# Z2PackDev/TBmodels

Hardware: AMD Instinct MI355X
Metric: k-points/sec (H(k)+eig) at N_orb=64, N_R=4096 (higher is better)
Workload: dtype f64; 1 GPU; cfg2: dense N_orb=64 N_R=4096, 100000 random k-points per GPU, eigenval (H(k)+eig); kpoints_per_gpu=100000, collective=none, rccl_ranks=0, eigensolver=auto

## Files before the change

include/tbk.h:

```cpp
#ifndef TBK_H
#define TBK_H

#include <stdint.h>

#ifdef __cplusplus
extern "C" {
#endif

typedef struct tbk_model tbk_model;
typedef struct tbk_kdotp tbk_kdotp;
typedef struct tbk_comm tbk_comm;

typedef enum tbk_status {
    TBK_OK = 0,
    TBK_ERR_ARGUMENT = 1,
    TBK_ERR_DEVICE = 2,
    TBK_ERR_MEMORY = 3,
    TBK_ERR_NOT_FINITE = 4,
    TBK_ERR_NO_CONVERGENCE = 5
} tbk_status;

enum { TBK_EIG_AUTO = 0, TBK_EIG_WAVE = 1, TBK_EIG_ROCSOLVER = 2 };
enum {
    TBK_OPT_EIGENSOLVER = 1,
    TBK_OPT_K_CHUNK = 2,
    TBK_OPT_TIMING = 3,
    TBK_OPT_FOLD = 4,
    TBK_OPT_STRASSEN = 5,
    TBK_OPT_STRASSEN_LEVELS = 6
};

const char* tbk_version(void);
const char* tbk_last_error(void);
int tbk_device_count(int* count);


int tbk_model_create_dense(int device, int dim, int n_orb, int64_t n_r, const int32_t* R,
                           const double* hop, tbk_model** out);

int tbk_model_create_csr(int device, int dim, int n_orb, int64_t n_r, const int32_t* R,
                         const int64_t* r_ptr, const int32_t* row, const int32_t* col,
                         const double* val, tbk_model** out);

void tbk_model_destroy(tbk_model* m);
int tbk_model_set_option(tbk_model* m, int option, int64_t value);
int tbk_model_info(const tbk_model* m, int* device, int* dim, int* n_orb, int64_t* n_r,
                   int* is_sparse, int64_t* staged_bytes);
enum { TBK_CNT_EIGENVAL_CALLS = 0, TBK_CNT_FOLDED_CALLS = 1, TBK_CNT_FOLDED_KPOINTS = 2,
       TBK_CNT_LIBRARY_CALLS = 3,
       TBK_CNT_STRASSEN_LAUNCHES = 4,
       TBK_CNT_STRASSEN2_LAUNCHES = 5,
       TBK_CNT_COUNT = 6 };
int tbk_model_counter(tbk_model* m, int counter, int64_t* value);


int tbk_hamilton(tbk_model* m, const double* k, int64_t nk, int convention, const double* pos,
                 double* H_out);

int tbk_eigenval(tbk_model* m, const double* k, int64_t nk, double* E_out);

int tbk_eigh(tbk_model* m, const double* k, int64_t nk, int convention, const double* pos, double* E_out, double* U_out);

int tbk_eigenval_multi(tbk_model* const* handles, int n_handles, const double* k, int64_t nk, double* E_out);
int tbk_hamilton_multi(tbk_model* const* handles, int n_handles, const double* k, int64_t nk, int convention,
                       const double* pos, double* H_out);
int tbk_eigh_multi(tbk_model* const* handles, int n_handles, const double* k, int64_t nk, int convention,
                   const double* pos, double* E_out, double* U_out);

int tbk_hamilton_device(tbk_model* m, const double* d_k, int64_t nk, int convention,
                        const double* d_pos, double* d_H);
int tbk_eigenval_device(tbk_model* m, const double* d_k, int64_t nk, double* d_E);
int tbk_eigh_device(tbk_model* m, const double* d_k, int64_t nk, int convention, const double* d_pos, double* d_E,
                    double* d_U);
int tbk_eigenval_device_hint(tbk_model* m, const double* d_k, const double* h_k, int64_t nk, double* d_E);
int tbk_eigenval_check(tbk_model* m);
int tbk_synchronize(tbk_model* m);

enum { TBK_REDUCE_AUTO = 0, TBK_REDUCE_ONE_STAGE = 1, TBK_REDUCE_TWO_STAGE = 2 };
int tbk_tridiagonal_reduce(int device, int n_orb, int64_t nk, const double* H, int method, double* d, double* e,
                           double* H_reduced);

int tbk_reduce_standalone(int device, int n_orb, int64_t nk, int reps, double* us_per_matrix);

int tbk_kdotp_create(int device, int dim, int n_orb, int64_t n_p, const int32_t* powers,
                     const double* coeffs, tbk_kdotp** out);
void tbk_kdotp_destroy(tbk_kdotp* m);
int tbk_kdotp_hamilton(tbk_kdotp* m, const double* k, int64_t nk, double* H_out);
int tbk_kdotp_eigenval(tbk_kdotp* m, const double* k, int64_t nk, double* E_out);
int tbk_kdotp_eigh(tbk_kdotp* m, const double* k, int64_t nk, double* E_out, double* U_out);
int tbk_kdotp_eigenval_multi(tbk_kdotp* const* handles, int n_handles, const double* k, int64_t nk, double* E_out);
int tbk_kdotp_hamilton_multi(tbk_kdotp* const* handles, int n_handles, const double* k, int64_t nk, double* H_out);
int tbk_kdotp_eigh_multi(tbk_kdotp* const* handles, int n_handles, const double* k, int64_t nk, double* E_out, double* U_out);

int tbk_kdotp_coefficients(tbk_model* m, const double* k0, int64_t n_p, const int32_t* powers,
                           const double* prefactor, double* coeffs_out);

int tbk_device_malloc(int device, int64_t bytes, void** d_ptr);
int tbk_device_free(int device, void* d_ptr);
int tbk_memcpy_h2d(int device, void* d_dst, const void* h_src, int64_t bytes);
int tbk_memcpy_d2h(int device, void* h_dst, const void* d_src, int64_t bytes);
int tbk_device_mem_info(int device, int64_t* free_bytes, int64_t* total_bytes);

enum { TBK_T_PHASE = 0, TBK_T_HK = 1, TBK_T_EIG = 2, TBK_T_QL = 3, TBK_T_COUNT = 4 };
int tbk_get_timing(tbk_model* m, double* ms, int64_t* launches, int reset);

int tbk_comm_unique_id(void* id128);
int tbk_comm_create(int device, int world_size, int rank, const void* id128, tbk_comm** out);
void tbk_comm_destroy(tbk_comm* c);
int tbk_comm_ranks(tbk_comm* c, int* count, int* rank);
int tbk_comm_allgather_f64(tbk_comm* c, tbk_model* m, const double* d_send, double* d_recv,
                           int64_t count);
int tbk_comm_allgather_f64_overlapped(tbk_comm* c, tbk_model* m, const double* d_send, double* d_recv,
                                      int64_t count, int slot);
int tbk_comm_wait_slot(tbk_comm* c, tbk_model* m, int slot);
int tbk_comm_synchronize(tbk_comm* c);
int tbk_comm_agree(tbk_comm* c, int status, double* verdict);
int tbk_comm_prepare_gather(tbk_comm* c, int n_orb, int64_t per);

int tbk_eigenval_device_gather(tbk_comm* c, tbk_model* m, const double* d_k, const double* h_k, int64_t nk, int64_t per,
                               int host_status, double* d_all, double* d_status_all);

int tbk_mfma_f64_peak(int device, double* tflops);

#ifdef __cplusplus
}
#endif
#endif
```

tbmodels_amd/_lib.py:

```python

import ctypes
import os

import numpy as np

_HERE = os.path.dirname(os.path.abspath(__file__))
LIB_PATH = os.environ.get("TBK_LIBTBK") or os.path.join(_HERE, "libtbk.so")

TBK_OK = 0
TBK_ERR_ARGUMENT = 1
TBK_ERR_DEVICE = 2
TBK_ERR_MEMORY = 3
TBK_ERR_NOT_FINITE = 4
TBK_ERR_NO_CONVERGENCE = 5

TBK_EIG_AUTO, TBK_EIG_WAVE, TBK_EIG_ROCSOLVER = 0, 1, 2
TBK_OPT_EIGENSOLVER, TBK_OPT_K_CHUNK, TBK_OPT_TIMING, TBK_OPT_FOLD, TBK_OPT_STRASSEN, TBK_OPT_STRASSEN_LEVELS = 1, 2, 3, 4, 5, 6
TBK_REDUCE_AUTO, TBK_REDUCE_ONE_STAGE, TBK_REDUCE_TWO_STAGE = 0, 1, 2
TBK_CNT_EIGENVAL_CALLS, TBK_CNT_FOLDED_CALLS, TBK_CNT_FOLDED_KPOINTS, TBK_CNT_LIBRARY_CALLS, TBK_CNT_STRASSEN_LAUNCHES = 0, 1, 2, 3, 4
TBK_CNT_STRASSEN2_LAUNCHES = 5
TBK_T_PHASE, TBK_T_HK, TBK_T_EIG, TBK_T_QL, TBK_T_COUNT = 0, 1, 2, 3, 4
STAGE_NAMES = ("phase", "hk", "eig", "ql")

_c_int = ctypes.c_int
_c_i64 = ctypes.c_int64
_vp = ctypes.c_void_p
_pp = ctypes.POINTER(ctypes.c_void_p)

SIGNATURES = {
    "tbk_version": (ctypes.c_char_p, []),
    "tbk_last_error": (ctypes.c_char_p, []),
    "tbk_device_count": (_c_int, [ctypes.POINTER(_c_int)]),
    "tbk_model_create_dense": (_c_int, [_c_int, _c_int, _c_int, _c_i64, _vp, _vp, _pp]),
    "tbk_model_create_csr": (_c_int, [_c_int, _c_int, _c_int, _c_i64, _vp, _vp, _vp, _vp, _vp, _pp]),
    "tbk_model_destroy": (None, [_vp]),
    "tbk_model_set_option": (_c_int, [_vp, _c_int, _c_i64]),
    "tbk_model_info": (
        _c_int,
        [_vp, ctypes.POINTER(_c_int), ctypes.POINTER(_c_int), ctypes.POINTER(_c_int), ctypes.POINTER(_c_i64),
         ctypes.POINTER(_c_int), ctypes.POINTER(_c_i64)],
    ),
    "tbk_hamilton": (_c_int, [_vp, _vp, _c_i64, _c_int, _vp, _vp]),
    "tbk_eigenval": (_c_int, [_vp, _vp, _c_i64, _vp]),
    "tbk_eigenval_multi": (_c_int, [_vp, _c_int, _vp, _c_i64, _vp]),
    "tbk_hamilton_multi": (_c_int, [_vp, _c_int, _vp, _c_i64, _c_int, _vp, _vp]),
    "tbk_eigh": (_c_int, [_vp, _vp, _c_i64, _c_int, _vp, _vp, _vp]),
    "tbk_eigh_multi": (_c_int, [_vp, _c_int, _vp, _c_i64, _c_int, _vp, _vp, _vp]),
    "tbk_eigh_device": (_c_int, [_vp, _vp, _c_i64, _c_int, _vp, _vp, _vp]),
    "tbk_hamilton_device": (_c_int, [_vp, _vp, _c_i64, _c_int, _vp, _vp]),
    "tbk_eigenval_device": (_c_int, [_vp, _vp, _c_i64, _vp]),
    "tbk_eigenval_device_hint": (_c_int, [_vp, _vp, _vp, _c_i64, _vp]),
    "tbk_model_counter": (_c_int, [_vp, _c_int, ctypes.POINTER(_c_i64)]),
    "tbk_eigenval_check": (_c_int, [_vp]),
    "tbk_synchronize": (_c_int, [_vp]),
    "tbk_tridiagonal_reduce": (_c_int, [_c_int, _c_int, _c_i64, _vp, _c_int, _vp, _vp, _vp]),
    "tbk_reduce_standalone": (_c_int, [_c_int, _c_int, _c_i64, _c_int, ctypes.POINTER(ctypes.c_double)]),
    "tbk_kdotp_create": (_c_int, [_c_int, _c_int, _c_int, _c_i64, _vp, _vp, _pp]),
    "tbk_kdotp_destroy": (None, [_vp]),
    "tbk_kdotp_hamilton": (_c_int, [_vp, _vp, _c_i64, _vp]),
    "tbk_kdotp_eigenval": (_c_int, [_vp, _vp, _c_i64, _vp]),
    "tbk_kdotp_eigenval_multi": (_c_int, [_vp, _c_int, _vp, _c_i64, _vp]),
    "tbk_kdotp_hamilton_multi": (_c_int, [_vp, _c_int, _vp, _c_i64, _vp]),
    "tbk_kdotp_eigh": (_c_int, [_vp, _vp, _c_i64, _vp, _vp]),
    "tbk_kdotp_eigh_multi": (_c_int, [_vp, _c_int, _vp, _c_i64, _vp, _vp]),
    "tbk_kdotp_coefficients": (_c_int, [_vp, _vp, _c_i64, _vp, _vp, _vp]),
    "tbk_device_malloc": (_c_int, [_c_int, _c_i64, _pp]),
    "tbk_device_free": (_c_int, [_c_int, _vp]),
    "tbk_memcpy_h2d": (_c_int, [_c_int, _vp, _vp, _c_i64]),
    "tbk_memcpy_d2h": (_c_int, [_c_int, _vp, _vp, _c_i64]),
    "tbk_device_mem_info": (_c_int, [_c_int, ctypes.POINTER(_c_i64), ctypes.POINTER(_c_i64)]),
    "tbk_get_timing": (_c_int, [_vp, ctypes.POINTER(ctypes.c_double), ctypes.POINTER(_c_i64), _c_int]),
    "tbk_comm_unique_id": (_c_int, [_vp]),
    "tbk_comm_create": (_c_int, [_c_int, _c_int, _c_int, _vp, _pp]),
    "tbk_comm_destroy": (None, [_vp]),
    "tbk_comm_ranks": (_c_int, [_vp, ctypes.POINTER(_c_int), ctypes.POINTER(_c_int)]),
    "tbk_comm_allgather_f64": (_c_int, [_vp, _vp, _vp, _vp, _c_i64]),
    "tbk_comm_allgather_f64_overlapped": (_c_int, [_vp, _vp, _vp, _vp, _c_i64, _c_int]),
    "tbk_comm_wait_slot": (_c_int, [_vp, _vp, _c_int]),
    "tbk_comm_synchronize": (_c_int, [_vp]),
    "tbk_comm_agree": (_c_int, [_vp, _c_int, _vp]),
    "tbk_comm_prepare_gather": (_c_int, [_vp, _c_int, _c_i64]),
    "tbk_eigenval_device_gather": (_c_int, [_vp, _vp, _vp, _vp, _c_i64, _c_i64, _c_int, _vp, _vp]),
    "tbk_mfma_f64_peak": (_c_int, [_c_int, ctypes.POINTER(ctypes.c_double)]),
}

_LIB = None


class TbkLibraryError(RuntimeError):
    """``libtbk.so`` is missing or cannot be loaded: the product path has no CPU fallback."""


def lib():
    global _LIB
    if _LIB is None:
        if not os.path.exists(LIB_PATH):
            raise TbkLibraryError(
                "{} not found: build it with `python -c 'import __graft_entry__ as g; g.build()'` "
                "(or `make -C tbmodels_amd/csrc`). There is no CPU fallback.".format(LIB_PATH)
            )
        try:
            handle = ctypes.CDLL(LIB_PATH, mode=ctypes.RTLD_GLOBAL)
        except OSError as exc:
            raise TbkLibraryError("cannot load {}: {}".format(LIB_PATH, exc)) from exc
        for name, (restype, argtypes) in SIGNATURES.items():
            func = getattr(handle, name)
            func.restype = restype
            func.argtypes = argtypes
        _LIB = handle
    return _LIB


def last_error():
    msg = lib().tbk_last_error()
    return msg.decode("utf-8", "replace") if msg else ""


def check(status):
    if status == TBK_OK:
        return
    msg = last_error()
    if status in (TBK_ERR_ARGUMENT, TBK_ERR_NOT_FINITE):
        raise ValueError(msg)
    if status == TBK_ERR_MEMORY:
        raise MemoryError(msg)
    if status == TBK_ERR_NO_CONVERGENCE:
        raise np.linalg.LinAlgError(msg)
    raise RuntimeError(msg)


def ptr(array):
    if array is None:
        return None
    assert array.flags.c_contiguous
    return array.__array_interface__["data"][0]


def device_count():
    count = ctypes.c_int(0)
    check(lib().tbk_device_count(ctypes.byref(count)))
    return count.value
```

tbmodels_amd/csrc/tbk_api.hip:

```cpp

#include <algorithm>
#include <cmath>
#include <cstdarg>
#include <cstdlib>
#include <cstring>
#include <dlfcn.h>
#include <functional>
#include <new>
#include <vector>

#include "tbk_internal.h"

static thread_local char g_err[1024] = "";

void tbk_set_error(const char* fmt, ...) {
    va_list ap;
    va_start(ap, fmt);
    vsnprintf(g_err, sizeof(g_err), fmt, ap);
    va_end(ap);
}

extern "C" const char* tbk_last_error(void) { return g_err; }
extern "C" const char* tbk_version(void) { return "tbk 0.1 (gfx950)"; }

extern "C" int tbk_device_count(int* count) {
    TBK_ARG(count != nullptr, "count is NULL");
    int n = 0;
    hipError_t e = hipGetDeviceCount(&n);
    if (e != hipSuccess) {
        (void)hipGetLastError();
        n = 0;
    }
    *count = n;
    return TBK_OK;
}

int DevBuf::reserve(size_t want) {
    if (want <= bytes) return TBK_OK;
    release();
    const size_t rounded = (want + (size_t(1) << 20) - 1) & ~((size_t(1) << 20) - 1);
    TBK_HIP(hipMalloc(&ptr, rounded));
    bytes = rounded;
    return TBK_OK;
}

void DevBuf::release() {
    if (ptr) (void)hipFree(ptr);
    ptr = nullptr;
    bytes = 0;
}

namespace {
struct RoctxApi {
    int (*push)(const char*) = nullptr;
    int (*pop)() = nullptr;
};
const RoctxApi& roctx_api() {
    static const RoctxApi api = [] {
        RoctxApi a;
        for (const char* name : {"librocprofiler-sdk-roctx.so", "librocprofiler-sdk-roctx.so.1", "libroctx64.so"}) {
            void* h = dlopen(name, RTLD_LAZY | RTLD_GLOBAL);
            if (!h) continue;
            a.push = reinterpret_cast<int (*)(const char*)>(dlsym(h, "roctxRangePushA"));
            a.pop = reinterpret_cast<int (*)()>(dlsym(h, "roctxRangePop"));
            if (a.push && a.pop) break;
            a.push = nullptr;
            a.pop = nullptr;
        }
        return a;
    }();
    return api;
}
const char* const kStageNames[TBK_T_COUNT] = {"tbk:phase_rows", "tbk:hk_contraction", "tbk:tridiag_reduction",
                                              "tbk:tridiag_eigenvalues"};
}

void tbk_range_push(const char* name) {
    const RoctxApi& api = roctx_api();
    if (api.push) (void)api.push(name);
}

void tbk_range_pop() {
    const RoctxApi& api = roctx_api();
    if (api.pop) (void)api.pop();
}

StageTimer::StageTimer(tbk_model* m_, int stage, hipStream_t s)
    : m(m_), on(m_->timing), stream(s ? s : m_->stream) {
    ev.stage = stage;
    if (on) {
        if (hipEventCreate(&ev.start) != hipSuccess || hipEventCreate(&ev.stop) != hipSuccess) {
            on = false;
            return;
        }
        tbk_range_push(kStageNames[stage]);
        (void)hipEventRecord(ev.start, stream);
    }
}

StageTimer::~StageTimer() {
    if (on) {
        (void)hipEventRecord(ev.stop, stream);
        tbk_range_pop();
        m->events.push_back(ev);
    }
}

static inline int64_t round_up(int64_t x, int64_t q) { return (x + q - 1) / q * q; }

static int require_device(int device) {
    int n = 0;
    if (hipGetDeviceCount(&n) != hipSuccess || n == 0) {
        (void)hipGetLastError();
        tbk_set_error("no HIP device visible: libtbk has no CPU path");
        return TBK_ERR_DEVICE;
    }
    if (device < 0 || device >= n) {
        tbk_set_error("device %d out of range (have %d)", device, n);
        return TBK_ERR_ARGUMENT;
    }
    TBK_HIP(hipSetDevice(device));
    return TBK_OK;
}

static int create_common(int device, int dim, int n_orb, int64_t n_r, const int32_t* R,
                         int64_t k_rows_per_r, bool pair_diagonal, tbk_model** out) {
    TBK_ARG(out != nullptr, "out is NULL");
    *out = nullptr;
    TBK_ARG(dim >= 1 && dim <= TBK_MAX_DIM, "dim must be in [1, 8]");
    TBK_ARG(n_orb >= 1 && n_orb <= 32768, "n_orb must be in [1, 32768]");
    TBK_ARG(n_r >= 0 && n_r < (int64_t(1) << 28), "n_r out of range");
    TBK_ARG(n_r == 0 || R != nullptr || k_rows_per_r == 1, "R is NULL");
    TBK_CHECK(require_device(device));

    tbk_model* m = new (std::nothrow) tbk_model();
    if (!m) {
        tbk_set_error("out of host memory");
        return TBK_ERR_MEMORY;
    }
    m->device = device;
    {
        int cus = 0;
        if (hipDeviceGetAttribute(&cus, hipDeviceAttributeMultiprocessorCount, device) == hipSuccess && cus > 0) m->n_cu = cus;
    }
    m->dim = dim;
    m->n_orb = n_orb;
    m->n_r = n_r;
    const bool strassen = pair_diagonal && k_rows_per_r == 2 && tbk_strassen_model(false, false, n_r);
    m->k2 = round_up(n_r * k_rows_per_r, strassen ? 2 * TBK_BK : TBK_BK);
    m->n_r_pad = m->k2 / k_rows_per_r;
    m->ncol = (int)(pair_diagonal ? (int64_t)n_orb * (n_orb - 1) / 2 + (n_orb + 1) / 2 : (int64_t)n_orb * (n_orb + 1) / 2);
    m->ncol_pad = (int)round_up(m->ncol, strassen ? 2 * TBK_BNP : TBK_BNP);

    int rc = TBK_OK;
    auto fail = [&](int code) {
        tbk_model_destroy(m);
        return code;
    };
#define TBK_TRY(expr)                           \
    do {                                        \
        rc = [&]() -> int {                     \
            expr;                               \
            return TBK_OK;                      \
        }();                                    \
        if (rc != TBK_OK) return fail(rc);      \
    } while (0)

    TBK_TRY(TBK_HIP(hipStreamCreateWithFlags(&m->stream, hipStreamNonBlocking)));
    TBK_TRY(TBK_HIP(hipStreamCreateWithFlags(&m->stream_eig, hipStreamNonBlocking)));
    TBK_TRY(TBK_HIP(hipStreamCreateWithFlags(&m->stream_ql, hipStreamNonBlocking)));
    for (int b = 0; b < 2; ++b) {
        TBK_TRY(TBK_HIP(hipEventCreateWithFlags(&m->ev_hk[b], hipEventDisableTiming)));
        TBK_TRY(TBK_HIP(hipEventCreateWithFlags(&m->ev_tri[b], hipEventDisableTiming)));
        TBK_TRY(TBK_HIP(hipEventCreateWithFlags(&m->ev_ql[b], hipEventDisableTiming)));
        TBK_TRY(TBK_HIP(hipEventCreateWithFlags(&m->ev_out[b], hipEventDisableTiming)));
        if (b == 0) TBK_TRY(TBK_HIP(hipEventCreateWithFlags(&m->ev_sync, hipEventDisableTiming | hipEventReleaseToSystem)));
    }
    TBK_TRY(TBK_ROCBLAS(rocblas_create_handle(&m->blas)));
    TBK_TRY(TBK_ROCBLAS(rocblas_set_stream(m->blas, m->stream)));
    TBK_TRY(TBK_CHECK(m->ws_flag.reserve(2 * sizeof(int))));
    TBK_TRY(TBK_HIP(hipMemsetAsync(m->ws_flag.ptr, 0, 2 * sizeof(int), m->stream)));
    m->h_stage_bytes = std::max<size_t>(size_t(320) << 10,
                                        n_orb <= 1024 ? (size_t)n_orb * n_orb * 16 + (size_t)n_orb * dim * 8 + (size_t(64) << 10) : 0);
    if (hipHostMalloc(&m->h_stage, m->h_stage_bytes, hipHostMallocNonCoherent) != hipSuccess) {
        (void)hipGetLastError();
        m->h_stage = nullptr;
        m->h_stage_bytes = 0;
    }

    {
        std::vector<int32_t> colmap((size_t)m->ncol_pad, -1);
        size_t e = 0;
        for (int i = 0; i < n_orb; ++i) {
            if (!pair_diagonal)
                colmap[e++] = (int32_t)((i << 16) | i);
            else if (i % 2 == 0)
                colmap[e++] = i + 1 < n_orb ? (int32_t)((i << 16) | TBK_SLOT_PAIR | (i + 1)) : (int32_t)((i << 16) | i);
            for (int j = i + 1; j < n_orb; ++j) colmap[e++] = (int32_t)((i << 16) | j);
        }
        TBK_TRY(TBK_HIP(hipMalloc((void**)&m->d_colmap, colmap.size() * sizeof(int32_t))));
        TBK_TRY(TBK_HIP(hipMemcpy(m->d_colmap, colmap.data(), colmap.size() * sizeof(int32_t),
                                  hipMemcpyHostToDevice)));
        m->staged_bytes += (int64_t)(colmap.size() * sizeof(int32_t));
    }
    if (n_r > 0 && R != nullptr && k_rows_per_r == 2) m->h_R.assign(R, R + (size_t)n_r * dim);
    if (m->n_r_pad > 0 && R != nullptr) {
        std::vector<int32_t> r_pad((size_t)m->n_r_pad * dim, 0);
        std::memcpy(r_pad.data(), R, (size_t)n_r * dim * sizeof(int32_t));
        TBK_TRY(TBK_HIP(hipMalloc((void**)&m->d_R, r_pad.size() * sizeof(int32_t))));
        TBK_TRY(TBK_HIP(hipMemcpy(m->d_R, r_pad.data(), r_pad.size() * sizeof(int32_t),
                                  hipMemcpyHostToDevice)));
        m->staged_bytes += (int64_t)(r_pad.size() * sizeof(int32_t));
    }
#undef TBK_TRY
    *out = m;
    return TBK_OK;
}

extern "C" int tbk_model_create_dense(int device, int dim, int n_orb, int64_t n_r, const int32_t* R,
                                      const double* hop, tbk_model** out) {
    TBK_ARG(out != nullptr, "out is NULL");
    *out = nullptr;
    TBK_ARG(n_r == 0 || hop != nullptr, "hop is NULL");
    tbk_model* m = nullptr;
    TBK_CHECK(create_common(device, dim, n_orb, n_r, R, 2, true, &m));
    m->sparse = false;
    int rc = TBK_OK;
    double* d_raw = nullptr;
    const size_t raw_bytes = (size_t)n_r * n_orb * n_orb * 2 * sizeof(double);
    rc = [&]() -> int {
        if (raw_bytes) {
            TBK_HIP(hipMalloc((void**)&d_raw, raw_bytes));
            TBK_HIP(hipMemcpyAsync(d_raw, hop, raw_bytes, hipMemcpyHostToDevice, m->stream));
        }
        TBK_CHECK(tbk_stage_dense(m, d_raw));
        TBK_CHECK(tbk_stage_strassen(m));
        TBK_HIP(hipStreamSynchronize(m->stream));
        return TBK_OK;
    }();
    if (d_raw) (void)hipFree(d_raw);
    if (rc != TBK_OK) {
        tbk_model_destroy(m);
        return rc;
    }
    *out = m;
    return TBK_OK;
}

extern "C" int tbk_model_create_csr(int device, int dim, int n_orb, int64_t n_r, const int32_t* R,
                                    const int64_t* r_ptr, const int32_t* row, const int32_t* col,
                                    const double* val, tbk_model** out) {
    TBK_ARG(out != nullptr, "out is NULL");
    *out = nullptr;
    TBK_ARG(n_r >= 0, "n_r out of range");
    TBK_ARG(n_r == 0 || r_ptr != nullptr, "r_ptr is NULL");
    const int64_t nnz = n_r > 0 ? r_ptr[n_r] : 0;
    TBK_ARG(n_r == 0 || r_ptr[0] == 0, "r_ptr[0] must be 0");
    TBK_ARG(nnz >= 0, "negative nnz");
    TBK_ARG(nnz == 0 || (row && col && val), "row/col/val is NULL");
    for (int64_t r = 0; r < n_r; ++r) TBK_ARG(r_ptr[r] <= r_ptr[r + 1], "r_ptr not monotone");
    for (int64_t t = 0; t < nnz; ++t)
        TBK_ARG(row[t] >= 0 && row[t] < n_orb && col[t] >= 0 && col[t] < n_orb,
                "row/col index out of range");

    tbk_model* m = nullptr;
    TBK_CHECK(create_common(device, dim, n_orb, n_r, R, 2, false, &m));
    m->sparse = true;

    auto packed_index = [n_orb](int i, int j) -> int64_t {
        return (int64_t)i * n_orb - (int64_t)i * (i - 1) / 2 + (j - i);
    };
    std::vector<int64_t> cptr((size_t)m->ncol + 1, 0);
    for (int64_t t = 0; t < nnz; ++t) {
        const int i = std::min(row[t], col[t]), j = std::max(row[t], col[t]);
        cptr[(size_t)packed_index(i, j) + 1]++;
    }
    for (int e = 0; e < m->ncol; ++e) cptr[(size_t)e + 1] += cptr[(size_t)e];
    std::vector<int32_t> rec_r((size_t)nnz);
    std::vector<double> rec_v((size_t)nnz * 2);
    {
        std::vector<int64_t> cursor(cptr.begin(), cptr.end() - 1);
        for (int64_t r = 0; r < n_r; ++r)
            for (int64_t t = r_ptr[r]; t < r_ptr[r + 1]; ++t) {
                const int i = row[t], j = col[t];
                const int kind = (i == j) ? 2 : (i < j ? 0 : 1);
                const int64_t e = packed_index(std::min(i, j), std::max(i, j));
                const int64_t slot = cursor[(size_t)e]++;
                rec_r[(size_t)slot] = (int32_t)((kind << 28) | (int32_t)r);
                rec_v[(size_t)slot * 2] = val[2 * t];
                rec_v[(size_t)slot * 2 + 1] = val[2 * t + 1];
            }
    }
    m->nnz_rec = nnz;
    int rc = [&]() -> int {
        TBK_HIP(hipMalloc((void**)&m->d_cptr, cptr.size() * sizeof(int64_t)));
        TBK_HIP(hipMemcpy(m->d_cptr, cptr.data(), cptr.size() * sizeof(int64_t), hipMemcpyHostToDevice));
        m->staged_bytes += (int64_t)(cptr.size() * sizeof(int64_t));
        if (nnz > 0) {
            TBK_HIP(hipMalloc((void**)&m->d_rec_r, (size_t)nnz * sizeof(int32_t)));
            TBK_HIP(hipMalloc((void**)&m->d_rec_v, (size_t)nnz * 2 * sizeof(double)));
            TBK_HIP(hipMemcpy(m->d_rec_r, rec_r.data(), (size_t)nnz * sizeof(int32_t), hipMemcpyHostToDevice));
            TBK_HIP(hipMemcpy(m->d_rec_v, rec_v.data(), (size_t)nnz * 2 * sizeof(double), hipMemcpyHostToDevice));
            m->staged_bytes += nnz * (int64_t)(sizeof(int32_t) + 2 * sizeof(double));
            const int kt = tbk_csr_tile_kpoints(n_r);
            if (kt > 0) {
                std::vector<int64_t> sptr;
                std::vector<int32_t> srec_r;
                std::vector<double> srec_v;
                tbk_csr_schedule(m->ncol, kt, cptr, rec_r, rec_v, sptr, srec_r, srec_v);
                m->sched_steps = sptr.back();
                auto upload = [&](void** dst, const void* src, size_t bytes) -> int {
                    TBK_HIP(hipMalloc(dst, std::max<size_t>(bytes, 8)));
                    if (bytes) TBK_HIP(hipMemcpy(*dst, src, bytes, hipMemcpyHostToDevice));
                    m->staged_bytes += (int64_t)bytes;
                    return TBK_OK;
                };
                TBK_CHECK(upload((void**)&m->d_sptr, sptr.data(), sptr.size() * sizeof(int64_t)));
                TBK_CHECK(upload((void**)&m->d_srec_r, srec_r.data(), srec_r.size() * sizeof(int32_t)));
                TBK_CHECK(upload((void**)&m->d_srec_v, srec_v.data(), srec_v.size() * sizeof(double)));
                m->sched_kt = kt;
            }
        }
        return TBK_OK;
    }();
    if (rc != TBK_OK) {
        tbk_model_destroy(m);
        return rc;
    }
    *out = m;
    return TBK_OK;
}

extern "C" void tbk_model_destroy(tbk_model* m) {
    if (!m) return;
    (void)hipSetDevice(m->device);
    hipStream_t streams[] = {m->stream, m->stream_eig, m->stream_ql, m->stream_xl[0], m->stream_xl[1], m->stream_xl[2]};
    for (hipStream_t st : streams)
        if (st) (void)hipStreamSynchronize(st);
    for (hipEvent_t e : m->ev_xl)
        if (e) (void)hipEventDestroy(e);
    for (int b = 0; b < 2; ++b) {
        if (m->ev_hk[b]) (void)hipEventDestroy(m->ev_hk[b]);
        if (m->ev_tri[b]) (void)hipEventDestroy(m->ev_tri[b]);
        if (m->ev_ql[b]) (void)hipEventDestroy(m->ev_ql[b]);
        if (m->ev_out[b]) (void)hipEventDestroy(m->ev_out[b]);
        if (b == 0 && m->ev_sync) (void)hipEventDestroy(m->ev_sync);
    }
    for (auto& ev : m->events) {
        (void)hipEventDestroy(ev.start);
        (void)hipEventDestroy(ev.stop);
    }
    if (m->blas) (void)rocblas_destroy_handle(m->blas);
    if (m->h_stage) (void)hipHostFree(m->h_stage);
    for (hipStream_t st : streams)
        if (st) (void)hipStreamDestroy(st);
    void* ptrs[] = {m->d_R, m->d_colmap, m->d_B, m->d_Bs, m->d_Bs2, m->d_cptr, m->d_rec_r, m->d_rec_v, m->d_powers, m->d_sptr, m->d_srec_r, m->d_srec_v};
    for (void* p : ptrs)
        if (p) (void)hipFree(p);
    DevBuf* bufs[] = {&m->ws_phase, &m->ws_H, &m->ws_E,   &m->ws_E2,
                      &m->ws_info,  &m->ws_k, &m->ws_pos, &m->ws_out, &m->ws_out2, &m->ws_flag, &m->ws_orb, &m->ws_part, &m->ws_kfold, &m->ws_kline, &m->ws_band, &m->ws_bandmat[0], &m->ws_bandmat[1], &m->ws_H2, &m->ws_xl, &m->ws_posraw};
    for (DevBuf* b : bufs) b->release();
    tbk_fold_release(m);
    delete m;
}

extern "C" int tbk_model_set_option(tbk_model* m, int option, int64_t value) {
    TBK_ARG(m != nullptr, "model is NULL");
    TBK_LOCK(m);
    switch (option) {
        case TBK_OPT_EIGENSOLVER:
            TBK_ARG(value >= TBK_EIG_AUTO && value <= TBK_EIG_ROCSOLVER, "unknown eigensolver");
            m->eigensolver = (int)value;
            return TBK_OK;
        case TBK_OPT_K_CHUNK:
            TBK_ARG(value >= 0, "k chunk must be >= 0");
            m->k_chunk = value;
            return TBK_OK;
        case TBK_OPT_TIMING:
            m->timing = value != 0;
            return TBK_OK;
        case TBK_OPT_FOLD:
            m->fold_enabled = value != 0;
            return TBK_OK;
        case TBK_OPT_STRASSEN:
            m->strassen = value != 0;
            return TBK_OK;
        case TBK_OPT_STRASSEN_LEVELS:
            TBK_ARG(value == 1 || value == 2, "Strassen levels must be 1 or 2");
            m->strassen_levels = (int)value;
            return TBK_OK;
        default:
            tbk_set_error("unknown option %d", option);
            return TBK_ERR_ARGUMENT;
    }
}

extern "C" int tbk_model_info(const tbk_model* m, int* device, int* dim, int* n_orb, int64_t* n_r,
                              int* is_sparse, int64_t* staged_bytes) {
    TBK_ARG(m != nullptr, "model is NULL");
    if (device) *device = m->device;
    if (dim) *dim = m->dim;
    if (n_orb) *n_orb = m->n_orb;
    if (n_r) *n_r = m->n_r;
    if (is_sparse) *is_sparse = m->sparse ? 1 : 0;
    if (staged_bytes) *staged_bytes = m->staged_bytes;
    return TBK_OK;
}

int64_t choose_chunk(tbk_model* m, int64_t nk, bool with_eig) {
    if (nk <= TBK_BM) return TBK_BM;
    const int64_t n = m->n_orb;
    int64_t per_k = m->k2 * 8 + (with_eig ? n * n * 16 + (int64_t)tbk_eig_scratch_per_k(m) : 0);
    if (per_k < 64) per_k = 64;
    size_t free_b = 0, total_b = 0;
    if (hipMemGetInfo(&free_b, &total_b) != hipSuccess) free_b = size_t(8) << 30;
    free_b += m->ws_H.bytes + m->ws_H2.bytes + m->ws_phase.bytes + m->ws_band.bytes + m->ws_bandmat[0].bytes + m->ws_bandmat[1].bytes +
              m->ws_E.bytes + m->ws_xl.bytes + m->ws_part.bytes;
    const bool mid = n > 64 && n <= 256;
    int64_t budget = std::min<int64_t>((int64_t)(free_b / 4), int64_t(mid ? 64 : n > 64 ? 24 : 6) << 30);
    int64_t chunk = budget / per_k / TBK_BM * TBK_BM;
    int64_t cap = mid ? 131072 : 32768;
    if (n < 64) cap *= std::min<int64_t>(32, (64 / n) * (64 / n));
    chunk = std::max<int64_t>(TBK_BM, std::min<int64_t>(chunk, cap));
    tbk_hk_plan_t plan = tbk_hk_plan(m, tbk_staged_operand(m), std::min(chunk, nk), false);
    if (plan.path == HK_PATH_STRASSEN2) {
        size_t free2 = free_b;
        if (m->d_Bs2 == nullptr) {
            const size_t blocks = tbk_strassen2_bytes(m);
            if (blocks > free_b / 4) m->bs2_skipped = true;
            else free2 -= blocks;
        }
        if (!m->bs2_skipped) {
            const int64_t per_k_s = per_k + m->k2 * 8 * 33 / 16 + (int64_t)m->ncol_pad * 16 * 49 / 16;
            const int64_t fit = (int64_t)(free2 / 4) / per_k_s / TBK_BM * TBK_BM;
            chunk = std::max<int64_t>(TBK_BM, std::min(chunk, fit));
        }
        plan = tbk_hk_plan(m, tbk_staged_operand(m), std::min(chunk, nk), false);
    }
    if (plan.path == HK_PATH_STRASSEN) {
        const int64_t per_k_s = per_k + m->k2 * 8 * 3 / 4 + (int64_t)m->ncol_pad * 16 * 7 / 4;
        const int64_t fit = (int64_t)(free_b / 4) / per_k_s / TBK_BM * TBK_BM;
        chunk = std::max<int64_t>(TBK_BM, std::min(chunk, fit));
    }
    if (m->k_chunk > 0) chunk = round_up(m->k_chunk, TBK_BM);
    else if (chunk >= 4096) chunk = chunk / 4096 * 4096;
    return std::min(chunk, round_up(nk, TBK_BM));
}

int fill_rows(tbk_model* m, const tbk_hk_plan_t& plan, const double* d_k) {
    TBK_CHECK(m->ws_phase.reserve((size_t)plan.row_doubles * sizeof(double)));
    double* d_A = m->ws_phase.as<double>();
    if (plan.rows == HK_ROWS_NONE) return TBK_OK;
    if (plan.rows == HK_ROWS_STRASSEN) return tbk_launch_phase_strassen(m, plan.op, d_k, plan.nk, d_A);
    if (plan.rows == HK_ROWS_STRASSEN2) {
        TBK_CHECK(tbk_stage_strassen2(m));
        return tbk_launch_phase_strassen2(m, plan.op, d_k, plan.nk, d_A);
    }
    if (plan.rows == HK_ROWS_MONOMIAL)
        return tbk_launch_monomials(m->stream, m->d_powers, plan.op.dim, plan.op.n_r, plan.op.k2, d_k, plan.nk, plan.nk_pad, d_A);
    return tbk_launch_phase(m, plan.op, d_k, plan.nk, plan.nk_pad, d_A);
}

int build_h(tbk_model* m, const tbk_hk_plan_t& plan, int mode, int convention, const double* d_k, const double* d_pos,
                   double* d_H) {
    const double* d_A = plan.rows == HK_ROWS_NONE ? nullptr : m->ws_phase.as<double>();
    if (plan.path == HK_PATH_CSR)
        return tbk_launch_hk_csr(m, d_A, plan.nk, plan.nk_pad, mode, convention, d_k, d_pos, d_H);
    return tbk_launch_hk_dense(m, plan, d_A, mode, convention, d_k, d_pos, d_H);
}

extern "C" int tbk_hamilton_device(tbk_model* m, const double* d_k, int64_t nk, int convention,
                                   const double* d_pos, double* d_H) {
    TBK_ARG(m != nullptr, "model is NULL");
    TBK_LOCK(m);
    TBK_ARG(convention == 1 || convention == 2, "convention must be 1 or 2");
    TBK_ARG(nk >= 0, "nk < 0");
    if (nk == 0) return TBK_OK;
    TBK_ARG(d_k && d_H, "k / H is NULL");
    TBK_ARG(convention == 2 || d_pos != nullptr, "convention 1 needs pos");
    TBK_HIP(hipSetDevice(m->device));
    const int64_t chunk = choose_chunk(m, nk, false);
    const size_t nn2 = (size_t)m->n_orb * m->n_orb * 2;
    for (int64_t c0 = 0; c0 < nk; c0 += chunk) {
        const int64_t nkc = std::min(chunk, nk - c0);
        const tbk_hk_plan_t plan = tbk_hk_plan(m, tbk_staged_operand(m), nkc, false);
        const double* kc = d_k + c0 * m->dim;
        TBK_CHECK(fill_rows(m, plan, kc));
        const double* d_orb = nullptr;
        const bool inline_orb = m->h_k_inline != nullptr && m->d_pos_inline != nullptr && nk == 1 && plan.rows == HK_ROWS_NONE;
        if (convention == 1 && !inline_orb) {
            TBK_CHECK(m->ws_orb.reserve((size_t)nkc * m->n_orb * 2 * sizeof(double)));
            TBK_CHECK(tbk_launch_orbital_phases(m, kc, d_pos, nkc, m->ws_orb.as<double>()));
            d_orb = m->ws_orb.as<double>();
        }
        TBK_CHECK(build_h(m, plan, HK_FULL, convention, kc, d_orb, d_H + (size_t)c0 * nn2));
    }
    return TBK_OK;
}

static int launch_tridiag_eigenvalues(tbk_model* m, const tbk_eig_plan_t& plan, hipStream_t s, double* d_de, int64_t nk, double* d_E,
                                      bool beside_ql = false, bool bisect_anyway = false, const void* d_band = nullptr) {
    if (d_band) TBK_CHECK(tbk_launch_band_chase(m, plan, s, d_band, nk, d_de));
    if (!plan.bisect && !bisect_anyway) return tbk_launch_ql(m, s, d_de, nk, d_E, beside_ql);
    return tbk_launch_bisect(m, plan, s, d_de, nk, d_E);
}

static std::vector<int64_t> chunk_schedule(tbk_model* m, int64_t nk, int64_t chunk) {
    std::vector<int64_t> out;
    const int64_t unit = 4096;
    if (!tbk_eig_small_supported(m->n_orb) || m->k_chunk > 0 || chunk < 2 * unit || nk < 3 * unit) {
        for (int64_t c0 = 0; c0 < nk; c0 += chunk) out.push_back(std::min(chunk, nk - c0));
        return out;
    }
    const int64_t last = unit + nk % unit;
    int64_t rest = nk - last;
    const int64_t n_big = (rest + chunk - 1) / chunk;
    for (int64_t i = 0; i < n_big; ++i) {
        const int64_t share = round_up((rest + (n_big - i) - 1) / (n_big - i), unit);
        const int64_t take = std::min(std::min(share, chunk), rest);
        out.push_back(take);
        rest -= take;
    }
    out.push_back(last);
    return out;
}

using HBuilder = std::function<int(int64_t c0, int64_t nkc, double* d_H)>;

static int eigenval_wave_pipeline(tbk_model* m, const tbk_eig_plan_t& plan, const double* d_k, int64_t nk, double* d_E,
                                  const HBuilder* builder = nullptr, const std::vector<int64_t>* runs = nullptr) {
    int64_t rows_ready_for = -1;
    tbk_hk_plan_t rows_plan;
    const auto prepare_rows = [&](int64_t c0, int64_t nkc) -> int {
        rows_plan = tbk_hk_plan(m, tbk_staged_operand(m), nkc, false);
        if (rows_plan.rows != HK_ROWS_NONE) TBK_CHECK(fill_rows(m, rows_plan, d_k + c0 * m->dim));
        rows_ready_for = c0;
        return TBK_OK;
    };
    const HBuilder direct = [&](int64_t c0, int64_t nkc, double* d_H) -> int {
        if (rows_ready_for != c0) TBK_CHECK(prepare_rows(c0, nkc));
        return build_h(m, rows_plan, HK_TRI, 2, d_k + c0 * m->dim, nullptr, d_H);
    };
    const HBuilder& build = builder ? *builder : direct;
    const int64_t chunk = choose_chunk(m, nk, true);
    const size_t n = (size_t)m->n_orb;
    const size_t nn2 = n * n * 2;
    DevBuf* debuf[2] = {&m->ws_E, &m->ws_E2};
    const std::vector<int64_t> sched =
        (runs != nullptr && m->k_chunk == 0 && nk > chunk) ? run_schedule(*runs, chunk) : chunk_schedule(m, nk, chunk);
    const int64_t n_chunks = (int64_t)sched.size();
    const int64_t max_chunk = *std::max_element(sched.begin(), sched.end());
    TBK_CHECK(m->ws_H.reserve((size_t)max_chunk * nn2 * sizeof(double)));
    for (int b = 0; b < (n_chunks > 1 ? 2 : 1); ++b)
        TBK_CHECK(debuf[b]->reserve((size_t)max_chunk * n * 2 * sizeof(double)));
    double* d_H = m->ws_H.as<double>();
    const bool h_overlap = n_chunks > 2 && builder != nullptr && plan.family == EIG_REGISTER;
    double* d_Hbuf[2] = {d_H, d_H};
    if (h_overlap) {
        TBK_CHECK(m->ws_H2.reserve((size_t)max_chunk * nn2 * sizeof(double)));
        d_Hbuf[1] = m->ws_H2.as<double>();
    }
    const bool two_stage = plan.family == EIG_TWO_STAGE && !plan.fused && n_chunks > 1;
    TBK_CHECK(tbk_eig_reserve(m, plan, max_chunk, n_chunks > 1 ? 2 : 1));
    if (n_chunks == 1) {
        double* d_de = debuf[0]->as<double>();
        TBK_CHECK(build(0, nk, d_H));
        TBK_CHECK(tbk_eig_reduce(m, plan, m->stream, d_H, nk, d_de));
        TBK_CHECK(launch_tridiag_eigenvalues(m, plan, m->stream, d_de, nk, d_E));
        if (m->chunk_done) {
            TBK_HIP(hipEventRecord(m->ev_ql[0], m->stream));
            TBK_CHECK(m->chunk_done(0, nk, m->ev_ql[0]));
        }
        return TBK_OK;
    }
    int64_t prev_c0 = 0, prev_nkc = 0, c0 = 0;
    for (int64_t c = 0; c < n_chunks; ++c) {
        const int b = (int)(c & 1);
        const int64_t nkc = sched[c];
        double* d_de = debuf[b]->as<double>();
        d_H = d_Hbuf[b];
        if (c >= 1) {
            if (!builder) TBK_CHECK(prepare_rows(c0, nkc));
            if (!h_overlap)
                TBK_HIP(hipStreamWaitEvent(m->stream, m->ev_tri[b ^ 1], 0));
            else if (c >= 2)
                TBK_HIP(hipStreamWaitEvent(m->stream, m->ev_tri[b], 0));
            if (c >= 2 && !h_overlap) TBK_HIP(hipStreamWaitEvent(m->stream, m->ev_ql[b], 0));
        }
        TBK_CHECK(build(c0, nkc, d_H));
        TBK_HIP(hipEventRecord(m->ev_hk[b], m->stream));

        TBK_HIP(hipStreamWaitEvent(m->stream_eig, m->ev_hk[b], 0));
        if (c >= 2 && h_overlap) TBK_HIP(hipStreamWaitEvent(m->stream_eig, m->ev_ql[b], 0));
        TBK_CHECK(tbk_eig_reduce(m, plan, m->stream_eig, d_H, nkc, d_de, two_stage ? m->ws_bandmat[b].ptr : nullptr));
        TBK_HIP(hipEventRecord(m->ev_tri[b], m->stream_eig));

        if (c >= 1) {
            TBK_HIP(hipStreamWaitEvent(m->stream_ql, m->ev_hk[b], 0));
            if (h_overlap) TBK_HIP(hipStreamWaitEvent(m->stream_ql, m->ev_tri[b ^ 1], 0));
            TBK_CHECK(launch_tridiag_eigenvalues(m, plan, m->stream_ql, debuf[b ^ 1]->as<double>(), prev_nkc,
                                                 d_E + (size_t)prev_c0 * n, false, false,
                                                 two_stage ? m->ws_bandmat[b ^ 1].ptr : nullptr));
            TBK_HIP(hipEventRecord(m->ev_ql[b ^ 1], m->stream_ql));
            if (m->chunk_done) TBK_CHECK(m->chunk_done(prev_c0, prev_nkc, m->ev_ql[b ^ 1]));
        }
        prev_c0 = c0;
        prev_nkc = nkc;
        c0 += nkc;
    }
    {
        const int b = (int)((n_chunks - 1) & 1);
        TBK_CHECK(launch_tridiag_eigenvalues(m, plan, m->stream_eig, debuf[b]->as<double>(), prev_nkc,
                                             d_E + (size_t)prev_c0 * n, true, true, two_stage ? m->ws_bandmat[b].ptr : nullptr));
        TBK_HIP(hipEventRecord(m->ev_ql[b], m->stream_eig));
        if (m->chunk_done) TBK_CHECK(m->chunk_done(prev_c0, prev_nkc, m->ev_ql[b]));
    }
    for (int b = 0; b < (n_chunks > 1 ? 2 : 1); ++b) TBK_HIP(hipStreamWaitEvent(m->stream, m->ev_ql[b], 0));
    TBK_HIP(hipStreamWaitEvent(m->stream, m->ev_tri[(n_chunks - 1) & 1], 0));
    return TBK_OK;
}

static int eigenval_folded(tbk_model* m, const tbk_eig_plan_t& eig_plan, const double* d_k, const double* h_k, int64_t nk, double* d_E,
                           bool* done) {
    *done = false;
    tbk_folded_call call(m, d_k, h_k, nk);
    if (!call.folds()) return TBK_OK;
    TBK_CHECK(call.begin());
    const HBuilder folded = [&call](int64_t c0, int64_t nkc, double* d_H) { return call.build(c0, nkc, d_H); };
    TBK_CHECK(eigenval_wave_pipeline(m, eig_plan, d_k, nk, d_E, &folded, &call.runs));
    m->counters[TBK_CNT_FOLDED_CALLS] += 1;
    m->counters[TBK_CNT_FOLDED_KPOINTS] += nk;
    *done = true;
    return TBK_OK;
}

__global__ void __launch_bounds__(256) flag_nonfinite_kernel(const double* __restrict__ E, int64_t total, int* __restrict__ flag) {
    bool bad = false;
    for (int64_t i = (int64_t)blockIdx.x * 256 + threadIdx.x; i < total; i += (int64_t)gridDim.x * 256) bad |= !isfinite(E[i]);
    if (__any(bad) && (threadIdx.x & 63) == 0) atomicAdd(flag, 1);
}

static int eigenval_device_impl(tbk_model* m, const tbk_eig_plan_t& plan, const double* d_k, const double* h_k, int64_t nk, double* d_E) {
    TBK_ARG(m != nullptr, "model is NULL");
    TBK_LOCK(m);
    TBK_ARG(nk >= 0, "nk < 0");
    if (nk == 0) return TBK_OK;
    TBK_ARG(d_k && d_E, "k / E is NULL");
    TBK_HIP(hipSetDevice(m->device));
    m->counters[TBK_CNT_EIGENVAL_CALLS] += 1;
    TBK_CHECK(tbk_eig_check_option(m));
    if (plan.own()) {
        bool done = false;
        TBK_CHECK(eigenval_folded(m, plan, d_k, h_k, nk, d_E, &done));
        if (done) return TBK_OK;
        return eigenval_wave_pipeline(m, plan, d_k, nk, d_E);
    }

    int64_t chunk = choose_chunk(m, nk, true);
    const size_t nn2 = (size_t)m->n_orb * m->n_orb * 2;
    chunk = std::max<int64_t>(1, std::min<int64_t>(chunk, (int64_t(1) << 29) / std::max<int64_t>(1, (int64_t)m->n_orb * m->n_orb)));
    m->counters[TBK_CNT_LIBRARY_CALLS] += 1;
    for (int64_t c0 = 0; c0 < nk; c0 += chunk) {
        const int64_t nkc = std::min(chunk, nk - c0);
        const tbk_hk_plan_t hk = tbk_hk_plan(m, tbk_staged_operand(m), nkc, true);
        const double* kc = d_k + c0 * m->dim;
        TBK_CHECK(fill_rows(m, hk, kc));
        TBK_CHECK(m->ws_H.reserve((size_t)nkc * nn2 * sizeof(double)));
        double* d_H = m->ws_H.as<double>();
        TBK_CHECK(build_h(m, hk, HK_TRI, 2, kc, nullptr, d_H));
        TBK_CHECK(tbk_eig_batched(m, d_H, nkc, d_E + (size_t)c0 * m->n_orb));
    }
    {
        const int64_t total = nk * m->n_orb;
        const unsigned blocks = (unsigned)std::min<int64_t>((total + 255) / 256, 8 * 1024);
        hipLaunchKernelGGL(flag_nonfinite_kernel, dim3(blocks), dim3(256), 0, m->stream, d_E, total, m->ws_flag.as<int>() + 1);
        TBK_HIP(hipGetLastError());
    }
    return TBK_OK;
}

extern "C" int tbk_eigenval_device_hint(tbk_model* m, const double* d_k, const double* h_k, int64_t nk, double* d_E) {
    TBK_ARG(m != nullptr, "model is NULL");
    TBK_LOCK(m);
    return eigenval_device_impl(m, tbk_eig_plan(m->n_orb, m->eigensolver, nk), d_k, h_k, nk, d_E);
}

extern "C" int tbk_eigenval_device(tbk_model* m, const double* d_k, int64_t nk, double* d_E) {
    return tbk_eigenval_device_hint(m, d_k, nullptr, nk, d_E);
}

extern "C" int tbk_model_counter(tbk_model* m, int counter, int64_t* value) {
    TBK_ARG(m != nullptr && value != nullptr, "model / value is NULL");
    TBK_ARG(counter >= 0 && counter < TBK_CNT_COUNT, "unknown counter");
    TBK_LOCK(m);
    *value = m->counters[counter];
    return TBK_OK;
}

static int wait_main_stream(tbk_model* m) {
    TBK_HIP(hipEventRecord(m->ev_sync, m->stream));
    TBK_HIP(hipEventSynchronize(m->ev_sync));
    return TBK_OK;
}

extern "C" int tbk_synchronize(tbk_model* m) {
    TBK_ARG(m != nullptr, "model is NULL");
    TBK_LOCK(m);
    TBK_HIP(hipSetDevice(m->device));
    return wait_main_stream(m);
}

extern "C" int tbk_eigenval_check(tbk_model* m) {
    TBK_ARG(m != nullptr, "model is NULL");
    TBK_LOCK(m);
    TBK_HIP(hipSetDevice(m->device));
    int flag[2] = {0, 0};
    TBK_HIP(hipMemcpyAsync(flag, m->ws_flag.ptr, sizeof(flag), hipMemcpyDeviceToHost, m->stream));
    TBK_HIP(hipMemsetAsync(m->ws_flag.ptr, 0, sizeof(flag), m->stream));
    TBK_CHECK(wait_main_stream(m));
    if (flag[1] != 0) {
        tbk_set_error("array must not contain infs or NaNs");
        return TBK_ERR_NOT_FINITE;
    }
    if (flag[0] != 0) {
        tbk_set_error("eigensolver did not converge for %d matrices", flag[0]);
        return TBK_ERR_NO_CONVERGENCE;
    }
    return TBK_OK;
}

extern "C" int tbk_hamilton(tbk_model* m, const double* k, int64_t nk, int convention,
                            const double* pos, double* H_out) {
    TBK_ARG(m != nullptr, "model is NULL");
    TBK_LOCK(m);
    TBK_ARG(convention == 1 || convention == 2, "convention must be 1 or 2");
    TBK_ARG(nk >= 0, "nk < 0");
    if (nk == 0) return TBK_OK;
    TBK_ARG(k && H_out, "k / H is NULL");
    TBK_ARG(convention == 2 || pos != nullptr, "convention 1 needs pos");
    TBK_HIP(hipSetDevice(m->device));
    const size_t nn2 = (size_t)m->n_orb * m->n_orb * 2;
    {
        const size_t k_bytes = (size_t)nk * m->dim * sizeof(double), h_bytes = (size_t)nk * nn2 * sizeof(double);
        const size_t p_bytes = convention == 1 ? (size_t)m->n_orb * m->dim * sizeof(double) : 0;
        const size_t h_off = (k_bytes + p_bytes + 63) / 64 * 64;
        if (m->h_stage != nullptr && h_off + h_bytes <= m->h_stage_bytes) {
            char* st = static_cast<char*>(m->h_stage);
            TBK_CHECK(m->ws_k.reserve(k_bytes));
            TBK_CHECK(m->ws_out.reserve(h_bytes));
            const bool inline_k = nk == 1 && tbk_hk_plan(m, tbk_staged_operand(m), 1, false).rows == HK_ROWS_NONE;
            const double* d_pos = nullptr;
            if (inline_k) {
                if (convention == 1) {
                    const size_t n_pos = (size_t)m->n_orb * m->dim;
                    if (m->pos_cache.size() != n_pos || std::memcmp(m->pos_cache.data(), pos, p_bytes) != 0) {
                        TBK_CHECK(m->ws_posraw.reserve(p_bytes));
                        std::memcpy(st + k_bytes, pos, p_bytes);
                        TBK_HIP(hipMemcpyAsync(m->ws_posraw.ptr, st + k_bytes, p_bytes, hipMemcpyHostToDevice, m->stream));
                        m->pos_cache.assign(pos, pos + n_pos);
                    }
                    m->d_pos_inline = m->ws_posraw.as<double>();
                    d_pos = m->d_pos_inline;
                }
                m->h_k_inline = k;
            } else {
                std::memcpy(st, k, k_bytes);
                TBK_HIP(hipMemcpyAsync(m->ws_k.ptr, st, k_bytes, hipMemcpyHostToDevice, m->stream));
                if (convention == 1) {
                    TBK_CHECK(m->ws_pos.reserve(p_bytes));
                    std::memcpy(st + k_bytes, pos, p_bytes);
                    TBK_HIP(hipMemcpyAsync(m->ws_pos.ptr, st + k_bytes, p_bytes, hipMemcpyHostToDevice, m->stream));
                    d_pos = m->ws_pos.as<double>();
                }
            }
            constexpr size_t ZERO_COPY_MAX = size_t(1) << 20;
            const bool direct = h_bytes <= ZERO_COPY_MAX;
            double* d_out = direct ? reinterpret_cast<double*>(st + h_off) : m->ws_out.as<double>();
            const int rc_inline = tbk_hamilton_device(m, m->ws_k.as<double>(), nk, convention, d_pos, d_out);
            m->h_k_inline = nullptr;
            m->d_pos_inline = nullptr;
            TBK_CHECK(rc_inline);
            if (!direct) TBK_HIP(hipMemcpyAsync(st + h_off, m->ws_out.ptr, h_bytes, hipMemcpyDeviceToHost, m->stream));
            TBK_CHECK(wait_main_stream(m));
            std::memcpy(H_out, st + h_off, h_bytes);
            return TBK_OK;
        }
    }
    const size_t total_bytes = (size_t)nk * nn2 * sizeof(double);
    const size_t chunk_bytes = std::min<size_t>(size_t(128) << 20, std::max<size_t>(size_t(16) << 20, total_bytes / 4));
    int64_t out_chunk = std::max<int64_t>(1, (int64_t)(chunk_bytes / (nn2 * sizeof(double))));
    out_chunk = std::min(out_chunk, nk);
    const int64_t n_chunks = (nk + out_chunk - 1) / out_chunk;
    TBK_CHECK(m->ws_k.reserve((size_t)nk * m->dim * sizeof(double)));
    TBK_HIP(hipMemcpyAsync(m->ws_k.ptr, k, (size_t)nk * m->dim * sizeof(double), hipMemcpyHostToDevice, m->stream));
    const double* d_pos = nullptr;
    if (convention == 1) {
        TBK_CHECK(m->ws_pos.reserve((size_t)m->n_orb * m->dim * sizeof(double)));
        TBK_HIP(hipMemcpyAsync(m->ws_pos.ptr, pos, (size_t)m->n_orb * m->dim * sizeof(double),
                               hipMemcpyHostToDevice, m->stream));
        d_pos = m->ws_pos.as<double>();
    }
    DevBuf* obuf[2] = {&m->ws_out, &m->ws_out2};
    for (int b = 0; b < (n_chunks > 1 ? 2 : 1); ++b) TBK_CHECK(obuf[b]->reserve((size_t)out_chunk * nn2 * sizeof(double)));
    auto compute = [&](int64_t c) -> int {
        const int64_t c0 = c * out_chunk, nkc = std::min(out_chunk, nk - c0);
        TBK_CHECK(tbk_hamilton_device(m, m->ws_k.as<double>() + c0 * m->dim, nkc, convention, d_pos, obuf[c & 1]->as<double>()));
        TBK_HIP(hipEventRecord(m->ev_out[c & 1], m->stream));
        return TBK_OK;
    };
    TBK_CHECK(compute(0));
    for (int64_t c = 0; c < n_chunks; ++c) {
        const int64_t c0 = c * out_chunk, nkc = std::min(out_chunk, nk - c0);
        if (c + 1 < n_chunks) TBK_CHECK(compute(c + 1));
        TBK_HIP(hipEventSynchronize(m->ev_out[c & 1]));
        TBK_HIP(hipMemcpy(H_out + (size_t)c0 * nn2, obuf[c & 1]->ptr, (size_t)nkc * nn2 * sizeof(double), hipMemcpyDeviceToHost));
    }
    return wait_main_stream(m);
}

__global__ void __launch_bounds__(256) export_small_kernel(const double* __restrict__ E, int64_t count, const int* __restrict__ flag,
                                                           double* __restrict__ host_E, int* __restrict__ host_flag) {
    for (int64_t i = (int64_t)blockIdx.x * 256 + threadIdx.x; i < count; i += (int64_t)gridDim.x * 256) host_E[i] = E[i];
    if (blockIdx.x == 0 && threadIdx.x < 2) host_flag[threadIdx.x] = flag[threadIdx.x];
}

extern "C" int tbk_eigenval(tbk_model* m, const double* k, int64_t nk, double* E_out) {
    TBK_ARG(m != nullptr, "model is NULL");
    TBK_LOCK(m);
    TBK_ARG(nk >= 0, "nk < 0");
    if (nk == 0) return TBK_OK;
    TBK_ARG(k && E_out, "k / E is NULL");
    TBK_HIP(hipSetDevice(m->device));
    const tbk_eig_plan_t plan = tbk_eig_plan(m->n_orb, m->eigensolver, nk);
    const size_t k_bytes = (size_t)nk * m->dim * sizeof(double), e_bytes = (size_t)nk * m->n_orb * sizeof(double);
    TBK_CHECK(m->ws_k.reserve(k_bytes));
    TBK_CHECK(m->ws_out.reserve(e_bytes));
    const size_t e_off = (k_bytes + 63) / 64 * 64;
    if (m->h_stage != nullptr && e_off + e_bytes + 16 <= m->h_stage_bytes) {
        char* st = static_cast<char*>(m->h_stage);
        int* flag = reinterpret_cast<int*>(st + e_off + e_bytes);
        const bool inline_k = nk == 1 && plan.own() && tbk_hk_plan(m, tbk_staged_operand(m), 1, false).rows == HK_ROWS_NONE;
        if (inline_k) {
            m->h_k_inline = k;
        } else {
            std::memcpy(st, k, k_bytes);
            TBK_HIP(hipMemcpyAsync(m->ws_k.ptr, st, k_bytes, hipMemcpyHostToDevice, m->stream));
        }
        const int rc_inline = eigenval_device_impl(m, plan, m->ws_k.as<double>(), k, nk, m->ws_out.as<double>());
        m->h_k_inline = nullptr;
        TBK_CHECK(rc_inline);
        {
            const int64_t count = nk * m->n_orb;
            const unsigned blocks = (unsigned)std::min<int64_t>((count + 255) / 256, 64);
            hipLaunchKernelGGL(export_small_kernel, dim3(blocks), dim3(256), 0, m->stream, m->ws_out.as<double>(), count,
                               m->ws_flag.as<int>(), reinterpret_cast<double*>(st + e_off), flag);
            TBK_HIP(hipGetLastError());
        }
        TBK_CHECK(wait_main_stream(m));
        std::memcpy(E_out, st + e_off, e_bytes);
        if (flag[0] != 0 || flag[1] != 0) return tbk_eigenval_check(m);
        return TBK_OK;
    }
    TBK_HIP(hipMemcpyAsync(m->ws_k.ptr, k, k_bytes, hipMemcpyHostToDevice, m->stream));
    TBK_CHECK(eigenval_device_impl(m, plan, m->ws_k.as<double>(), k, nk, m->ws_out.as<double>()));
    TBK_HIP(hipMemcpyAsync(E_out, m->ws_out.ptr, e_bytes, hipMemcpyDeviceToHost, m->stream));
    return tbk_eigenval_check(m);
}

extern "C" int tbk_tridiagonal_reduce(int device, int n_orb, int64_t nk, const double* H, int method, double* d, double* e,
                                      double* H_reduced) {
    TBK_ARG(nk >= 0, "nk < 0");
    TBK_ARG(n_orb >= 1 && (n_orb <= 64 || tbk_eig_band_supported(n_orb)),
            "n_orb must be in [1, 4096] (larger matrices go through rocSOLVER as a whole)");
    TBK_ARG(method >= TBK_REDUCE_AUTO && method <= TBK_REDUCE_TWO_STAGE, "unknown reduction method");
    TBK_ARG(method != TBK_REDUCE_TWO_STAGE || tbk_eig_band_supported(n_orb), "the two-stage reduction handles 64 < n_orb <= 4096");
    TBK_ARG(method != TBK_REDUCE_ONE_STAGE || n_orb <= 512, "the one-stage reduction handles n_orb <= 512");
    if (nk == 0) return TBK_OK;
    TBK_ARG(H && d && e, "H / d / e is NULL");
    tbk_model* m = nullptr;
    TBK_CHECK(create_common(device, 1, n_orb, 0, nullptr, 2, false, &m));
    const size_t n = (size_t)n_orb, mat_bytes = n * n * 2 * sizeof(double);
    int rc = [&]() -> int {
        TBK_LOCK(m);
        const tbk_eig_plan_t plan = tbk_eig_plan(n_orb, m->eigensolver, nk, method);
        TBK_CHECK(m->ws_H.reserve((size_t)nk * mat_bytes));
        TBK_CHECK(m->ws_E.reserve((size_t)nk * n * 2 * sizeof(double)));
        TBK_CHECK(tbk_eig_reserve(m, plan, nk, 1));
        TBK_HIP(hipMemcpyAsync(m->ws_H.ptr, H, (size_t)nk * mat_bytes, hipMemcpyHostToDevice, m->stream));
        TBK_CHECK(tbk_eig_reduce(m, plan, m->stream, m->ws_H.as<double>(), nk, m->ws_E.as<double>()));
        TBK_HIP(hipMemcpyAsync(d, m->ws_E.ptr, (size_t)nk * n * sizeof(double), hipMemcpyDeviceToHost, m->stream));
        TBK_HIP(hipMemcpyAsync(e, m->ws_E.as<double>() + (size_t)nk * n, (size_t)nk * n * sizeof(double), hipMemcpyDeviceToHost,
                               m->stream));
        if (H_reduced)
            TBK_HIP(hipMemcpyAsync(H_reduced, m->ws_H.ptr, (size_t)nk * mat_bytes, hipMemcpyDeviceToHost, m->stream));
        TBK_HIP(hipStreamSynchronize(m->stream));
        return TBK_OK;
    }();
    tbk_model_destroy(m);
    return rc;
}

__global__ void __launch_bounds__(256) random_hermitian_kernel(double* __restrict__ H, int n, int64_t nk) {
    const int64_t total = nk * (int64_t)n * n;
    for (int64_t t = (int64_t)blockIdx.x * 256 + threadIdx.x; t < total; t += (int64_t)gridDim.x * 256) {
        const int64_t mat = t / ((int64_t)n * n);
        const int r = (int)((t / n) % n), c = (int)(t % n);
        const int i = r < c ? r : c, j = r < c ? c : r;
        uint64_t x = (uint64_t)mat * 0x9E3779B97F4A7C15ull + (uint64_t)i * 0xBF58476D1CE4E5B9ull + (uint64_t)j * 0x94D049BB133111EBull + 1;
        x ^= x >> 30; x *= 0xBF58476D1CE4E5B9ull; x ^= x >> 27; x *= 0x94D049BB133111EBull; x ^= x >> 31;
        const double re = (double)(int64_t)(x >> 11) * (1.0 / 9007199254740992.0) - 0.5;
        x ^= x >> 29; x *= 0x9E3779B97F4A7C15ull; x ^= x >> 32;
        const double im = (double)(int64_t)(x >> 11) * (1.0 / 9007199254740992.0) - 0.5;
        H[2 * t] = re;
        H[2 * t + 1] = i == j ? 0.0 : (r < c ? im : -im);
    }
}

extern "C" int tbk_reduce_standalone(int device, int n_orb, int64_t nk, int reps, double* us_per_matrix) {
    TBK_ARG(us_per_matrix != nullptr, "us_per_matrix is NULL");
    TBK_ARG(nk >= 1 && reps >= 1, "nk / reps < 1");
    TBK_ARG(n_orb >= 1 && (n_orb <= 64 || tbk_eig_band_supported(n_orb)), "n_orb must be in [1, 4096]");
    for (int q = 0; q < 3; ++q) us_per_matrix[q] = 0.0;
    tbk_model* m = nullptr;
    TBK_CHECK(create_common(device, 1, n_orb, 0, nullptr, 2, false, &m));
    const size_t n = (size_t)n_orb, mat_bytes = n * n * 2 * sizeof(double);
    DevBuf pristine;
    hipEvent_t ev[2] = {nullptr, nullptr};
    int rc = [&]() -> int {
        TBK_LOCK(m);
        const tbk_eig_plan_t plan = tbk_eig_plan(n_orb, m->eigensolver, nk);
        TBK_CHECK(pristine.reserve((size_t)nk * mat_bytes));
        TBK_CHECK(m->ws_H.reserve((size_t)nk * mat_bytes));
        TBK_CHECK(m->ws_E.reserve((size_t)nk * n * 2 * sizeof(double)));
        TBK_HIP(hipEventCreate(&ev[0]));
        TBK_HIP(hipEventCreate(&ev[1]));
        hipLaunchKernelGGL(random_hermitian_kernel, dim3(4096), dim3(256), 0, m->stream, pristine.as<double>(), n_orb, nk);
        TBK_HIP(hipGetLastError());
        const bool band = plan.family == EIG_TWO_STAGE;
        TBK_CHECK(tbk_eig_reserve(m, plan, nk, 1));
        TBK_CHECK(m->ws_bandmat[0].reserve((size_t)nk * plan.band_stride));
        for (int what = 0; what < (band ? 3 : 1); ++what) {
            float sum = 0.0f;
            for (int r = 0; r <= reps; ++r) {
                if (what != 2)
                    TBK_HIP(hipMemcpyAsync(m->ws_H.ptr, pristine.ptr, (size_t)nk * mat_bytes, hipMemcpyDeviceToDevice, m->stream));
                TBK_HIP(hipEventRecord(ev[0], m->stream));
                if (what == 0) {
                    TBK_CHECK(tbk_eig_reduce(m, plan, m->stream, m->ws_H.as<double>(), nk, m->ws_E.as<double>()));
                } else if (what == 1) {
                    TBK_CHECK(tbk_launch_band_reduce(m, plan, m->stream, m->ws_H.as<double>(), nk, m->ws_band.ptr, m->ws_bandmat[0].ptr));
                } else {
                    TBK_CHECK(tbk_launch_band_chase(m, plan, m->stream, m->ws_bandmat[0].ptr, nk, m->ws_E.as<double>()));
                }
                TBK_HIP(hipEventRecord(ev[1], m->stream));
                TBK_HIP(hipEventSynchronize(ev[1]));
                float ms = 0.0f;
                TBK_HIP(hipEventElapsedTime(&ms, ev[0], ev[1]));
                if (r > 0) sum += ms;
            }
            us_per_matrix[what] = (double)sum / reps * 1e3 / (double)nk;
        }
        return TBK_OK;
    }();
    for (auto& e : ev)
        if (e) (void)hipEventDestroy(e);
    pristine.release();
    tbk_model_destroy(m);
    return rc;
}

extern "C" int tbk_kdotp_create(int device, int dim, int n_orb, int64_t n_p, const int32_t* powers,
                                const double* coeffs, tbk_kdotp** out) {
    TBK_ARG(out != nullptr, "out is NULL");
    *out = nullptr;
    TBK_ARG(n_p == 0 || (powers && coeffs), "powers / coeffs is NULL");
    for (int64_t t = 0; t < n_p * dim; ++t) TBK_ARG(powers[t] >= 0, "negative power");
    tbk_model* m = nullptr;
    TBK_CHECK(create_common(device, dim, n_orb, n_p, nullptr, 1, false, &m));
    m->kdotp = true;
    double* d_raw = nullptr;
    const size_t raw_bytes = (size_t)n_p * n_orb * n_orb * 2 * sizeof(double);
    int rc = [&]() -> int {
        if (n_p > 0) {
            TBK_HIP(hipMalloc((void**)&m->d_powers, (size_t)n_p * dim * sizeof(int32_t)));
            TBK_HIP(hipMemcpy(m->d_powers, powers, (size_t)n_p * dim * sizeof(int32_t), hipMemcpyHostToDevice));
            TBK_HIP(hipMalloc((void**)&d_raw, raw_bytes));
            TBK_HIP(hipMemcpyAsync(d_raw, coeffs, raw_bytes, hipMemcpyHostToDevice, m->stream));
        }
        TBK_CHECK(tbk_stage_kdotp(m, d_raw));
        TBK_HIP(hipStreamSynchronize(m->stream));
        return TBK_OK;
    }();
    if (d_raw) (void)hipFree(d_raw);
    if (rc != TBK_OK) {
        tbk_model_destroy(m);
        return rc;
    }
    tbk_kdotp* kp = new (std::nothrow) tbk_kdotp();
    if (!kp) {
        tbk_model_destroy(m);
        tbk_set_error("out of host memory");
        return TBK_ERR_MEMORY;
    }
    kp->core = m;
    *out = kp;
    return TBK_OK;
}

extern "C" void tbk_kdotp_destroy(tbk_kdotp* kp) {
    if (!kp) return;
    tbk_model_destroy(kp->core);
    delete kp;
}

extern "C" int tbk_kdotp_hamilton(tbk_kdotp* kp, const double* k, int64_t nk, double* H_out) {
    TBK_ARG(kp != nullptr, "model is NULL");
    return tbk_hamilton(kp->core, k, nk, 2, nullptr, H_out);
}

extern "C" int tbk_kdotp_eigenval(tbk_kdotp* kp, const double* k, int64_t nk, double* E_out) {
    TBK_ARG(kp != nullptr, "model is NULL");
    return tbk_eigenval(kp->core, k, nk, E_out);
}

extern "C" int tbk_device_malloc(int device, int64_t bytes, void** d_ptr) {
    TBK_ARG(d_ptr != nullptr && bytes >= 0, "bad malloc arguments");
    TBK_CHECK(require_device(device));
    *d_ptr = nullptr;
    if (bytes == 0) return TBK_OK;
    TBK_HIP(hipMalloc(d_ptr, (size_t)bytes));
    return TBK_OK;
}

extern "C" int tbk_device_free(int device, void* d_ptr) {
    if (!d_ptr) return TBK_OK;
    TBK_CHECK(require_device(device));
    TBK_HIP(hipFree(d_ptr));
    return TBK_OK;
}

extern "C" int tbk_memcpy_h2d(int device, void* d_dst, const void* h_src, int64_t bytes) {
    TBK_CHECK(require_device(device));
    if (bytes > 0) {
        TBK_HIP(hipMemcpy(d_dst, h_src, (size_t)bytes, hipMemcpyHostToDevice));
        TBK_HIP(hipDeviceSynchronize());
    }
    return TBK_OK;
}

extern "C" int tbk_memcpy_d2h(int device, void* h_dst, const void* d_src, int64_t bytes) {
    TBK_CHECK(require_device(device));
    if (bytes > 0) TBK_HIP(hipMemcpy(h_dst, d_src, (size_t)bytes, hipMemcpyDeviceToHost));
    return TBK_OK;
}

extern "C" int tbk_device_mem_info(int device, int64_t* free_bytes, int64_t* total_bytes) {
    TBK_CHECK(require_device(device));
    size_t f = 0, t = 0;
    TBK_HIP(hipMemGetInfo(&f, &t));
    if (free_bytes) *free_bytes = (int64_t)f;
    if (total_bytes) *total_bytes = (int64_t)t;
    return TBK_OK;
}

extern "C" int tbk_get_timing(tbk_model* m, double* ms, int64_t* launches, int reset) {
    TBK_ARG(m != nullptr, "model is NULL");
    TBK_LOCK(m);
    TBK_HIP(hipSetDevice(m->device));
    TBK_HIP(hipStreamSynchronize(m->stream));
    TBK_HIP(hipStreamSynchronize(m->stream_eig));
    TBK_HIP(hipStreamSynchronize(m->stream_ql));
    for (auto& ev : m->events) {
        float t = 0.f;
        if (hipEventElapsedTime(&t, ev.start, ev.stop) == hipSuccess) {
            m->t_ms[ev.stage] += (double)t;
            m->t_n[ev.stage] += 1;
        }
        (void)hipEventDestroy(ev.start);
        (void)hipEventDestroy(ev.stop);
    }
    m->events.clear();
    for (int i = 0; i < TBK_T_COUNT; ++i) {
        if (ms) ms[i] = m->t_ms[i];
        if (launches) launches[i] = m->t_n[i];
        if (reset) {
            m->t_ms[i] = 0.0;
            m->t_n[i] = 0;
        }
    }
    return TBK_OK;
}

extern "C" int tbk_mfma_f64_peak(int device, double* tflops) {
    TBK_ARG(tflops != nullptr, "tflops is NULL");
    TBK_CHECK(require_device(device));
    return tbk_run_mfma_f64_peak(tflops);
}
```

tbmodels_amd/csrc/tbk_hk_dense.hip:

```cpp

#include <algorithm>
#include <cstdlib>
#include <type_traits>

#include "tbk_internal.h"

namespace {

typedef double d4 __attribute__((ext_vector_type(4)));
typedef double d2 __attribute__((ext_vector_type(2)));
typedef __attribute__((address_space(1))) const void* gptr_t;
typedef __attribute__((address_space(3))) void* lptr_t;

constexpr int LDA = TBK_BM + 16;
constexpr int LDB = 2 * TBK_BNP + 16;
constexpr int STAGE_DOUBLES = TBK_BK * (LDA + LDB);

static_assert(TBK_BM == 128 && TBK_BNP == 64 && TBK_BK == 16, "wave decomposition is written for 128x64x16");

struct HkArgs {
    const double* A = nullptr;
    const double* Bt = nullptr;
    const int32_t* colmap = nullptr;
    const double* kpts = nullptr;
    const int32_t* R = nullptr;
    int64_t n_r = 0;
    const double* pos = nullptr;
    double* H = nullptr;
    int64_t k2 = 0;
    int64_t nk = 0;
    int64_t nk_pad = 0;
    int ncol_pad = 0;
    int n_orb = 0;
    int dim = 0;
    int mt_count = 0;
    int nt_count = 0;
    int xcd_rows = 0;
    double* P = nullptr;
    int splits = 1;
    int unit_grid = 1;
    int64_t p_rows = 0;
    int products = 0;
    int64_t a_prod_stride = 0, b_prod_stride = 0;
    int64_t a_tile_stride = TBK_BM;
    int64_t b_tile_stride = 0;
    int rows_per_tile = TBK_BM;
    int block_offset = 0;
    int p_tiles = 0;
    int sub_splits = 1;
    double* P2 = nullptr;
    double k_val[TBK_MAX_DIM] = {};
    int k_inline = 0;
    const double* pos_raw = nullptr;
};

__device__ __forceinline__ double hk_kcomp(const HkArgs& a, int64_t kq, int d) { return a.k_inline ? a.k_val[d] : a.kpts[kq * a.dim + d]; }

template <int MODE, int CONV>
__device__ __forceinline__ void store_element(const HkArgs& a, int64_t kq, int oi, int oj, double re, double im) {
    if (CONV == 1 && oi != oj) {
        d2 ei, ej;
        if (a.k_inline) {
            double di = 0.0, dj = 0.0;
            for (int d = 0; d < a.dim; ++d) {
                di = fma(a.k_val[d], a.pos_raw[oi * a.dim + d], di);
                dj = fma(a.k_val[d], a.pos_raw[oj * a.dim + d], dj);
            }
            double sn, cs;
            sincospi(2.0 * di, &sn, &cs);
            ei = (d2){cs, sn};
            sincospi(2.0 * dj, &sn, &cs);
            ej = (d2){cs, sn};
        } else {
            ei = *reinterpret_cast<const d2*>(a.pos + ((size_t)kq * a.n_orb + oi) * 2);
            ej = *reinterpret_cast<const d2*>(a.pos + ((size_t)kq * a.n_orb + oj) * 2);
        }
        const double cs = ei[0] * ej[0] + ei[1] * ej[1], sn = ei[0] * ej[1] - ei[1] * ej[0];
        const double t = re * cs - im * sn;
        im = re * sn + im * cs;
        re = t;
    }
    double* hk = a.H + (size_t)kq * a.n_orb * a.n_orb * 2;
    *reinterpret_cast<d2*>(hk + ((size_t)oi * a.n_orb + oj) * 2) = (d2){re, im};
    if (MODE == HK_FULL && oi != oj) *reinterpret_cast<d2*>(hk + ((size_t)oj * a.n_orb + oi) * 2) = (d2){re, -im};
}

template <int MODE, int CONV>
__device__ __forceinline__ void store_slot(const HkArgs& a, int64_t kq, int32_t slot, double v0, double v1) {
    const int oi = slot >> 16, oj = slot & 0x7fff;
    if (slot & TBK_SLOT_PAIR) {
        double* hk = a.H + (size_t)kq * a.n_orb * a.n_orb * 2;
        *reinterpret_cast<d2*>(hk + ((size_t)oi * a.n_orb + oi) * 2) = (d2){v0, 0.0};
        *reinterpret_cast<d2*>(hk + ((size_t)oj * a.n_orb + oj) * 2) = (d2){v1, 0.0};
        return;
    }
    store_element<MODE, CONV>(a, kq, oi, oj, v0, v1);
}

__device__ __forceinline__ bool tile_of_block(const HkArgs& a, int b, int& mt, int& nt) {
    if (a.xcd_rows == 0) {
        nt = b % a.nt_count;
        mt = b / a.nt_count;
        return mt < a.mt_count;
    }
    const int x = b & 7;
    const int t = b >> 3;
    const int base = a.mt_count >> 3, extra = a.mt_count & 7;
    const int rows = base + (x < extra ? 1 : 0);
    if (t >= rows * a.nt_count) return false;
    const int start = x * base + (x < extra ? x : extra);
    const int full = rows / a.xcd_rows;
    const int per_group = a.xcd_rows * a.nt_count;
    int row;
    if (t < full * per_group) {
        const int g = t / per_group, r = t % per_group;
        row = g * a.xcd_rows + r % a.xcd_rows;
        nt = r / a.xcd_rows;
    } else {
        const int tt = t - full * per_group, rr = rows - full * a.xcd_rows;
        row = full * a.xcd_rows + tt % rr;
        nt = tt / rr;
    }
    mt = start + row;
    return true;
}

template <int MODE, int CONV, bool SPLIT>
__global__ void __launch_bounds__(256, 2) hk_dense_kernel(const HkArgs a) {
    extern __shared__ __attribute__((aligned(16))) double smem[];

    const int unit = (int)blockIdx.x + a.block_offset;
    const int split_y = SPLIT ? unit / a.unit_grid : 0;
    int mt_idx, nt_idx;
    if (!tile_of_block(a, SPLIT ? unit - split_y * a.unit_grid : unit, mt_idx, nt_idx)) return;

    const int tid = threadIdx.x;
    const int lane = tid & 63;
    const int wave = __builtin_amdgcn_readfirstlane(tid >> 6);
    const int wm = wave >> 1;
    const int wn = wave & 1;
    const int l15 = lane & 15;
    const int l4 = lane >> 4;

    const int64_t m0 = (int64_t)mt_idx * a.rows_per_tile;
    const int64_t n0 = (int64_t)nt_idx * TBK_BNP;

    d4 acc[4][2][2];
#pragma unroll
    for (int i = 0; i < 4; ++i)
#pragma unroll
        for (int j = 0; j < 2; ++j)
#pragma unroll
            for (int p = 0; p < 2; ++p) acc[i][j][p] = (d4){0.0, 0.0, 0.0, 0.0};

    const double* opA = a.A;
    const double* opB = a.Bt;
    int s_begin = 0, n_stage = (int)(a.k2 / TBK_BK);
    if (SPLIT && a.products) {
        opA += split_y * a.a_prod_stride;
        opB += split_y * a.b_prod_stride;
    } else if (SPLIT) {
        const int per = (n_stage + a.splits - 1) / a.splits;
        s_begin = min(split_y * per, n_stage);
        n_stage = min(s_begin + per, n_stage);
        if (a.p_tiles > 0) {
            const int per2 = (n_stage - s_begin + a.sub_splits - 1) / a.sub_splits;
            s_begin = min(s_begin + (int)blockIdx.y * per2, n_stage);
            n_stage = min(s_begin + per2, n_stage);
        }
    }

    const uint32_t lane_bytes = (uint32_t)lane * 16u;
    const int64_t ldgA = a.nk_pad * (int64_t)sizeof(double);
    const int64_t ldgB = (int64_t)a.ncol_pad * 2 * (int64_t)sizeof(double);
    const char* rowA = reinterpret_cast<const char*>(opA + (int64_t)mt_idx * a.a_tile_stride) + ((int64_t)s_begin * TBK_BK + wave) * ldgA;
    const char* rowB = reinterpret_cast<const char*>(opB + (int64_t)mt_idx * a.b_tile_stride + n0 * 2) + ((int64_t)s_begin * TBK_BK + wave) * ldgB;
    auto issue_stage = [&](auto bufc) {
        constexpr int buf = decltype(bufc)::value;
        double* sA = smem + buf * STAGE_DOUBLES + wave * LDA;
        double* sB = smem + buf * STAGE_DOUBLES + TBK_BK * LDA + wave * LDB;
        uint32_t off = lane_bytes;
        asm volatile("" : "+v"(off));
#pragma unroll
        for (int i = 0; i < 4; ++i) {
            __builtin_amdgcn_global_load_lds((gptr_t)(rowA + (int64_t)(4 * i) * ldgA + off), (lptr_t)(sA + 4 * i * LDA), 16, 0, 0);
            __builtin_amdgcn_global_load_lds((gptr_t)(rowB + (int64_t)(4 * i) * ldgB + off), (lptr_t)(sB + 4 * i * LDB), 16, 0, 0);
        }
        rowA += TBK_BK * ldgA;
        rowB += TBK_BK * ldgB;
    };
    typedef __attribute__((address_space(3))) const double* lds_cptr;
    uint32_t fragA[2][TBK_BK / 4], fragB[2][TBK_BK / 4];
    {
        const uint32_t s0 = (uint32_t)(uintptr_t)(lptr_t)smem;
#pragma unroll
        for (int buf = 0; buf < 2; ++buf)
#pragma unroll
            for (int ks = 0; ks < TBK_BK / 4; ++ks) {
                fragA[buf][ks] = s0 + 8u * (uint32_t)(buf * STAGE_DOUBLES + wm * 64 + l15 + (ks * 4 + l4) * LDA);
                fragB[buf][ks] = s0 + 8u * (uint32_t)(buf * STAGE_DOUBLES + TBK_BK * LDA + wn * 64 + l15 + (ks * 4 + l4) * LDB);
                asm volatile("" : "+v"(fragA[buf][ks]), "+v"(fragB[buf][ks]));
            }
    }
    struct Frags {
        double fa[4], fb[2][2];
    };
    auto read_frags = [&](auto bufc, auto ksc) -> Frags {
        constexpr int buf = decltype(bufc)::value, ks = decltype(ksc)::value;
        const lds_cptr sA = (lds_cptr)(uintptr_t)fragA[buf][ks];
        const lds_cptr sB = (lds_cptr)(uintptr_t)fragB[buf][ks];
        Frags f;
#pragma unroll
        for (int i = 0; i < 4; ++i) f.fa[i] = sA[i * 16];
#pragma unroll
        for (int j = 0; j < 2; ++j) {
            f.fb[j][0] = sB[j * 32];
            f.fb[j][1] = sB[j * 32 + 16];
        }
        return f;
    };
    auto mfma_step = [&](const Frags& f) {
#pragma unroll
        for (int i = 0; i < 4; ++i)
#pragma unroll
            for (int j = 0; j < 2; ++j) {
                acc[i][j][0] = __builtin_amdgcn_mfma_f64_16x16x4f64(f.fa[i], f.fb[j][0], acc[i][j][0], 0, 0, 0);
                acc[i][j][1] = __builtin_amdgcn_mfma_f64_16x16x4f64(f.fa[i], f.fb[j][1], acc[i][j][1], 0, 0, 0);
            }
    };
    using buf0 = std::integral_constant<int, 0>;
    using buf1 = std::integral_constant<int, 1>;
    using ks0 = std::integral_constant<int, 0>;
    using ks1 = std::integral_constant<int, 1>;
    using ks2 = std::integral_constant<int, 2>;
    using ks3 = std::integral_constant<int, 3>;
    static_assert(TBK_BK == 16, "four K steps per stage are written out below");
    auto stage = [&](auto bufc, auto nextc, Frags& cur, bool more) {
        Frags f1 = read_frags(bufc, ks1{});
        mfma_step(cur);
        Frags f2 = read_frags(bufc, ks2{});
        mfma_step(f1);
        Frags f3 = read_frags(bufc, ks3{});
        mfma_step(f2);
        __syncthreads();
        if (more) cur = read_frags(nextc, ks0{});
        mfma_step(f3);
    };

    const int left = n_stage - s_begin;
    if (left > 0) issue_stage(buf0{});
    __syncthreads();
    Frags cur = read_frags(buf0{}, ks0{});
    for (int pair = 0; pair < (left >> 1); ++pair) {
        issue_stage(buf1{});
        stage(buf0{}, buf1{}, cur, true);
        const bool more = 2 * pair + 2 < left;
        if (more) issue_stage(buf0{});
        stage(buf1{}, buf0{}, cur, more);
    }
    if (left & 1) stage(buf0{}, buf1{}, cur, false);

#pragma unroll
    for (int j = 0; j < 2; ++j) {
        const int e = (int)n0 + (wn * 2 + j) * 16 + l15;
        const int32_t ij = a.colmap[e];
        if (ij < 0 && !(SPLIT && a.products)) continue;
#pragma unroll
        for (int i = 0; i < 4; ++i) {
#pragma unroll
            for (int r = 0; r < 4; ++r) {
                const int local = wm * 64 + i * 16 + l4 + 4 * r;
                const int64_t kq = m0 + local;
                if (local >= a.rows_per_tile || kq >= a.nk) continue;
                if (SPLIT) {
                    double* part =
                        a.p_tiles > 0
                            ? a.P2 + ((((size_t)blockIdx.y * a.p_tiles + blockIdx.x) * TBK_BM + local) * TBK_BNP +
                                      (wn * 2 + j) * 16 + l15) * 2
                            : a.P + (((size_t)split_y * a.p_rows + kq) * a.ncol_pad + e) * 2;
                    *reinterpret_cast<d2*>(part) = (d2){acc[i][j][0][r], acc[i][j][1][r]};
                } else {
                    store_slot<MODE, CONV>(a, kq, ij, acc[i][j][0][r], acc[i][j][1][r]);
                }
            }
        }
    }
}

constexpr int GEMV_U = 8;

template <int NKV, bool INLINE_PHASES>
__global__ void __launch_bounds__(256) hk_gemv_kernel(const HkArgs a, int strip_doubles) {
    extern __shared__ __attribute__((aligned(16))) double s_rows[];
    constexpr int U = NKV >= 32 ? 4 : GEMV_U;
    const int lane = threadIdx.x & 63;
    const int wave = __builtin_amdgcn_readfirstlane(threadIdx.x >> 6);
    const int nblk = a.ncol_pad >> 6;
    const int b = (int)blockIdx.x, n_wg = (int)gridDim.x;
    const int xcd = b & 7, per_xcd = n_wg >> 3, extra = n_wg & 7;
    const int wg = xcd * per_xcd + min(xcd, extra) + (b >> 3);
    const int task = wg * 4 + wave;
    const int sl = task / nblk, cb = task - sl * nblk;
    if (sl >= a.splits) return;
    const int64_t n_pairs = a.k2 >> 1;
    const int64_t kk0 = 2 * (sl * n_pairs / a.splits);
    const int n_rows = (int)(2 * ((sl + 1) * n_pairs / a.splits) - kk0);
    const int64_t kbase = (int64_t)blockIdx.z * NKV;
    const int nk_here = (int)min((int64_t)NKV, a.nk - kbase);
    const int64_t ld2 = a.ncol_pad;
    const d2* rows = reinterpret_cast<const d2*>(a.Bt) + kk0 * ld2 + cb * 64;
    double* strip = s_rows + wave * strip_doubles;

    d2 buf0[U], buf1[U];
    double acc[NKV][2];
#pragma unroll
    for (int q = 0; q < NKV; ++q) acc[q][0] = acc[q][1] = 0.0;

    auto fetch = [&](d2 (&buf)[U], int base) {
#pragma unroll
        for (int u = 0; u < U; ++u) {
            const int r = min(base + u, n_rows - 1);
            buf[u] = __builtin_nontemporal_load(rows + (int64_t)r * ld2 + lane);
        }
    };
    auto consume = [&](const d2 (&buf)[U], int row) {
        const double* arow = INLINE_PHASES ? strip + row * NKV : a.A + (kk0 + row) * a.nk_pad + kbase;
        const int64_t lda = INLINE_PHASES ? NKV : a.nk_pad;
#pragma unroll
        for (int u = 0; u < U; ++u) {
            if (!INLINE_PHASES && row + u >= n_rows) break;
#pragma unroll
            for (int q = 0; q < NKV; ++q) {
                const double aq = arow[u * lda + q];
                acc[q][0] = fma(aq, buf[u][0], acc[q][0]);
                acc[q][1] = fma(aq, buf[u][1], acc[q][1]);
            }
        }
    };
    fetch(buf0, 0);
    fetch(buf1, U);
    if (INLINE_PHASES) {
        for (int idx = lane; idx < ((n_rows + 15) >> 4) * 8 * NKV; idx += 64) {
            const int rr = idx / NKV, q = idx % NKV;
            const int64_t r = (kk0 >> 1) + rr;
            double sn = 0.0, cs = 0.0;
            if (q < nk_here && r < a.n_r && 2 * rr < n_rows) {
                double dot = 0.0;
                for (int d = 0; d < a.dim; ++d) dot = fma(hk_kcomp(a, kbase + q, d), (double)a.R[r * a.dim + d], dot);
                sincospi(2.0 * dot, &sn, &cs);
            }
            strip[(2 * rr) * NKV + q] = cs;
            strip[(2 * rr + 1) * NKV + q] = sn;
        }
        asm volatile("s_waitcnt lgkmcnt(0)" ::: "memory");
    }
    for (int row = 0; row < n_rows; row += 2 * U) {
        consume(buf0, row);
        __builtin_amdgcn_sched_barrier(0);
        fetch(buf0, row + 2 * U);
        __builtin_amdgcn_sched_barrier(0);
        consume(buf1, row + U);
        __builtin_amdgcn_sched_barrier(0);
        fetch(buf1, row + 3 * U);
        __builtin_amdgcn_sched_barrier(0);
    }
    const bool hi = (lane & 8) != 0;
    const int e = cb * 64 + (lane >> 4) * 16 + (lane & 7) * 2 + (hi ? 1 : 0);
#pragma unroll
    for (int q = 0; q < NKV; ++q) {
        const double got = __shfl_xor(hi ? acc[q][0] : acc[q][1], 8, 64);
        if (q < nk_here) {
            double* part = a.P + (((size_t)sl * a.p_rows + kbase + q) * a.ncol_pad + e) * 2;
            *reinterpret_cast<d2*>(part) = hi ? (d2){got, acc[q][1]} : (d2){acc[q][0], got};
        }
    }
}

template <int MODE, int CONV>
__global__ void __launch_bounds__(256) hk_tiny_kernel(const HkArgs a, int strip_doubles) {
    extern __shared__ __attribute__((aligned(16))) double s_tiny[];
    const int lane = threadIdx.x & 63;
    const int wave = __builtin_amdgcn_readfirstlane(threadIdx.x >> 6);
    const int cb = blockIdx.x;
    const int64_t n_pairs = a.k2 >> 1;
    const int64_t kk0 = 2 * (wave * n_pairs / 4);
    const int n_rows = (int)(2 * ((wave + 1) * n_pairs / 4) - kk0);
    const int64_t ld2 = a.ncol_pad;
    const d2* rows = reinterpret_cast<const d2*>(a.Bt) + kk0 * ld2 + cb * 64;
    double* strip = s_tiny + wave * strip_doubles;
    d2* part = reinterpret_cast<d2*>(s_tiny + 4 * strip_doubles);
    d2 buf0[GEMV_U], buf1[GEMV_U];
    auto fetch = [&](d2 (&buf)[GEMV_U], int base) {
#pragma unroll
        for (int u = 0; u < GEMV_U; ++u) buf[u] = rows[(int64_t)min(base + u, n_rows - 1) * ld2 + lane];
    };
    fetch(buf0, 0);
    fetch(buf1, GEMV_U);
    for (int rr = lane; rr < ((n_rows + 15) >> 4) * 8; rr += 64) {
        const int64_t r = (kk0 >> 1) + rr;
        double sn = 0.0, cs = 0.0;
        if (r < a.n_r && 2 * rr < n_rows) {
            double dot = 0.0;
            for (int d = 0; d < a.dim; ++d) dot = fma(hk_kcomp(a, 0, d), (double)a.R[r * a.dim + d], dot);
            sincospi(2.0 * dot, &sn, &cs);
        }
        strip[2 * rr] = cs;
        strip[2 * rr + 1] = sn;
    }
    asm volatile("s_waitcnt lgkmcnt(0)" ::: "memory");
    double acc0 = 0.0, acc1 = 0.0;
    auto consume = [&](const d2 (&buf)[GEMV_U], int row) {
#pragma unroll
        for (int u = 0; u < GEMV_U; ++u) {
            const double aq = strip[row + u];
            acc0 = fma(aq, buf[u][0], acc0);
            acc1 = fma(aq, buf[u][1], acc1);
        }
    };
    for (int row = 0; row < n_rows; row += 2 * GEMV_U) {
        consume(buf0, row);
        __builtin_amdgcn_sched_barrier(0);
        fetch(buf0, row + 2 * GEMV_U);
        __builtin_amdgcn_sched_barrier(0);
        consume(buf1, row + GEMV_U);
        __builtin_amdgcn_sched_barrier(0);
        fetch(buf1, row + 3 * GEMV_U);
        __builtin_amdgcn_sched_barrier(0);
    }
    const bool hi = (lane & 8) != 0;
    const int el = (lane >> 4) * 16 + (lane & 7) * 2 + (hi ? 1 : 0);
    const double got = __shfl_xor(hi ? acc0 : acc1, 8, 64);
    part[wave * 64 + el] = hi ? (d2){got, acc1} : (d2){acc0, got};
    __syncthreads();
    if (wave != 0) return;
    const int e = cb * 64 + lane;
    const int32_t ij = a.colmap[e];
    if (ij < 0) return;
    d2 sum = part[lane];
#pragma unroll
    for (int w = 1; w < 4; ++w) {
        sum[0] += part[w * 64 + lane][0];
        sum[1] += part[w * 64 + lane][1];
    }
    store_slot<MODE, CONV>(a, 0, ij, sum[0], sum[1]);
}

template <int MODE, int CONV>
__global__ void __launch_bounds__(256) hk_finish_kernel(const HkArgs a) {
    const int64_t idx = (int64_t)blockIdx.x * 256 + threadIdx.x;
    const int e = (int)(idx % a.ncol_pad);
    const int64_t kq = idx / a.ncol_pad;
    if (kq >= a.nk) return;
    const int32_t ij = a.colmap[e];
    if (ij < 0) return;
    double re = 0.0, im = 0.0;
    for (int sp = 0; sp < a.splits; ++sp) {
        const d2 v = *reinterpret_cast<const d2*>(a.P + (((size_t)sp * a.p_rows + kq) * a.ncol_pad + e) * 2);
        re += v[0];
        im += v[1];
    }
    store_slot<MODE, CONV>(a, kq, ij, re, im);
}

template <int MODE, int CONV>
__global__ void __launch_bounds__(256) hk_strassen_finish_kernel(const HkArgs a, int64_t mh) {
    const int half = a.ncol_pad / 2;
    const int64_t idx = (int64_t)blockIdx.x * 256 + threadIdx.x;
    const int e = (int)(idx % half);
    const int64_t kq = idx / half;
    if (kq >= mh) return;
    const size_t blk = (size_t)mh * half;
    const d2* mp = reinterpret_cast<const d2*>(a.P) + (size_t)kq * half + e;
    const d2 m1 = mp[0], m2 = mp[blk], m3 = mp[2 * blk], m4 = mp[3 * blk], m5 = mp[4 * blk], m6 = mp[5 * blk], m7 = mp[6 * blk];
    const d2 c11 = ((m1 + m4) - m5) + m7;
    const d2 c12 = m3 + m5;
    const d2 c21 = m2 + m4;
    const d2 c22 = ((m1 - m2) + m3) + m6;
    const int32_t ij0 = a.colmap[e], ij1 = a.colmap[e + half];
    if (kq < a.nk) {
        if (ij0 >= 0) store_slot<MODE, CONV>(a, kq, ij0, c11[0], c11[1]);
        if (ij1 >= 0) store_slot<MODE, CONV>(a, kq, ij1, c12[0], c12[1]);
    }
    if (kq + mh < a.nk) {
        if (ij0 >= 0) store_slot<MODE, CONV>(a, kq + mh, ij0, c21[0], c21[1]);
        if (ij1 >= 0) store_slot<MODE, CONV>(a, kq + mh, ij1, c22[0], c22[1]);
    }
}

template <int MODE, int CONV>
__global__ void __launch_bounds__(256) hk_strassen2_finish_kernel(const HkArgs a, int64_t mq) {
    const int quarter = a.ncol_pad / 4;
    const int64_t idx = (int64_t)blockIdx.x * 256 + threadIdx.x;
    const int e = (int)(idx % quarter);
    const int64_t kq = idx / quarter;
    if (kq >= mq) return;
    const size_t blk = (size_t)mq * quarter;
    const d2* mp = reinterpret_cast<const d2*>(a.P) + (size_t)kq * quarter + e;
    d2 c[2][2][2][2];
#pragma unroll
    for (int p1 = 0; p1 < 7; ++p1) {
        const d2* q = mp + (size_t)(7 * p1) * blk;
        const d2 m1 = q[0], m2 = q[blk], m3 = q[2 * blk], m4 = q[3 * blk], m5 = q[4 * blk], m6 = q[5 * blk], m7 = q[6 * blk];
        const d2 in[2][2] = {{((m1 + m4) - m5) + m7, m3 + m5}, {m2 + m4, ((m1 - m2) + m3) + m6}};
#pragma unroll
        for (int a2 = 0; a2 < 2; ++a2)
#pragma unroll
            for (int c2 = 0; c2 < 2; ++c2) {
                const d2 v = in[a2][c2];
                if (p1 == 0) c[0][0][a2][c2] = v, c[1][1][a2][c2] = v;
                if (p1 == 1) c[1][0][a2][c2] = v, c[1][1][a2][c2] -= v;
                if (p1 == 2) c[0][1][a2][c2] = v, c[1][1][a2][c2] += v;
                if (p1 == 3) c[0][0][a2][c2] += v, c[1][0][a2][c2] += v;
                if (p1 == 4) c[0][0][a2][c2] -= v, c[0][1][a2][c2] += v;
                if (p1 == 5) c[1][1][a2][c2] += v;
                if (p1 == 6) c[0][0][a2][c2] += v;
            }
    }
#pragma unroll
    for (int cq = 0; cq < 4; ++cq) {
        const int32_t ij = a.colmap[e + cq * quarter];
        if (ij < 0) continue;
#pragma unroll
        for (int aq = 0; aq < 4; ++aq) {
            const int64_t kout = kq + aq * mq;
            if (kout >= a.nk) continue;
            const d2 v = c[aq >> 1][cq >> 1][aq & 1][cq & 1];
            store_slot<MODE, CONV>(a, kout, ij, v[0], v[1]);
        }
    }
}

template <int MODE, int CONV>
__global__ void __launch_bounds__(256) hk_finish_wide_kernel(const HkArgs a) {
    __shared__ double part[4][16][2];
    const int lane = threadIdx.x & 63, wave = threadIdx.x >> 6;
    const int el = lane & 15;
    const int j = wave * 4 + (lane >> 4);
    const int64_t idx = (int64_t)blockIdx.x * 16 + el;
    const int e = (int)(idx % a.ncol_pad);
    const int64_t kq = idx / a.ncol_pad;
    double re = 0.0, im = 0.0;
    if (kq < a.nk)
        for (int sp = j; sp < a.splits; sp += 16) {
            const d2 v = *reinterpret_cast<const d2*>(a.P + (((size_t)sp * a.p_rows + kq) * a.ncol_pad + e) * 2);
            re += v[0];
            im += v[1];
        }
    re += __shfl_xor(re, 16, 64);
    im += __shfl_xor(im, 16, 64);
    re += __shfl_xor(re, 32, 64);
    im += __shfl_xor(im, 32, 64);
    if (lane < 16) {
        part[wave][el][0] = re;
        part[wave][el][1] = im;
    }
    __syncthreads();
    if (threadIdx.x < 16 && kq < a.nk) {
        const int32_t ij = a.colmap[e];
        if (ij < 0) return;
        const double sr = (part[0][el][0] + part[1][el][0]) + (part[2][el][0] + part[3][el][0]);
        const double si = (part[0][el][1] + part[1][el][1]) + (part[2][el][1] + part[3][el][1]);
        store_slot<MODE, CONV>(a, kq, ij, sr, si);
    }
}

template <int MODE, int CONV>
__global__ void __launch_bounds__(256) hk_finish_tiles_kernel(const HkArgs a) {
    const int unit = (int)blockIdx.x + a.block_offset;
    const int split_y = unit / a.unit_grid;
    int mt_idx, nt_idx;
    if (!tile_of_block(a, unit - split_y * a.unit_grid, mt_idx, nt_idx)) return;
    const int el = threadIdx.x & (TBK_BNP - 1);
    const int e = nt_idx * TBK_BNP + el;
    const int32_t ij = a.colmap[e];
    if (ij < 0) return;
    for (int local = threadIdx.x / TBK_BNP; local < a.rows_per_tile; local += 256 / TBK_BNP) {
        const int64_t kq = (int64_t)mt_idx * a.rows_per_tile + local;
        if (kq >= a.nk) break;
        double re = 0.0, im = 0.0;
        for (int sp = 0; sp < a.sub_splits; ++sp) {
            const d2 v = *reinterpret_cast<const d2*>(
                a.P2 + ((((size_t)sp * a.p_tiles + blockIdx.x) * TBK_BM + local) * TBK_BNP + el) * 2);
            re += v[0];
            im += v[1];
        }
        if (a.splits > 1)
            *reinterpret_cast<d2*>(a.P + (((size_t)split_y * a.p_rows + kq) * a.ncol_pad + e) * 2) = (d2){re, im};
        else
            store_slot<MODE, CONV>(a, kq, ij, re, im);
    }
}

template <int MODE, int CONV>
hipError_t launch_gemv(tbk_model* m, const HkArgs& a, size_t lds, hipStream_t s) {
    const int tasks = (a.ncol_pad >> 6) * a.splits;
    const dim3 grid((unsigned)((tasks + 3) / 4), 1, (unsigned)((a.nk + 31) / 32));
    static std::atomic<bool> raised[2][6][TBK_MAX_DEVICES] = {};
#define TBK_GEMV(N, SLOT)                                                                                               \
    do {                                                                                                                \
        if (a.A == nullptr) {                                                                                           \
            hipError_t e1 = tbk_raise_lds_limit(reinterpret_cast<const void*>(&hk_gemv_kernel<N, true>), 160 * 1024, raised[0][SLOT]); \
            if (e1 != hipSuccess) return e1;                                                                            \
            hipLaunchKernelGGL((hk_gemv_kernel<N, true>), grid, dim3(256), lds, s, a, (int)(lds / 32));                                  \
        } else {                                                                                                        \
            hipError_t e1 = tbk_raise_lds_limit(reinterpret_cast<const void*>(&hk_gemv_kernel<N, false>), 160 * 1024, raised[1][SLOT]); \
            if (e1 != hipSuccess) return e1;                                                                            \
            hipLaunchKernelGGL((hk_gemv_kernel<N, false>), grid, dim3(256), lds, s, a, (int)(lds / 32));                                 \
        }                                                                                                               \
    } while (0)
    if (a.nk <= 1)
        TBK_GEMV(1, 0);
    else if (a.nk <= 2)
        TBK_GEMV(2, 1);
    else if (a.nk <= 4)
        TBK_GEMV(4, 2);
    else if (a.nk <= 8)
        TBK_GEMV(8, 3);
    else if (a.nk <= 16)
        TBK_GEMV(16, 4);
    else
        TBK_GEMV(32, 5);
#undef TBK_GEMV
    (void)m;
    hipError_t e = hipGetLastError();
    if (e != hipSuccess) return e;
    const int64_t threads = a.nk * a.ncol_pad;
    if (a.splits >= 32)
        hipLaunchKernelGGL((hk_finish_wide_kernel<MODE, CONV>), dim3((unsigned)((threads + 15) / 16)), dim3(256), 0, s, a);
    else
        hipLaunchKernelGGL((hk_finish_kernel<MODE, CONV>), dim3((unsigned)((threads + 255) / 256)), dim3(256), 0, s, a);
    return hipGetLastError();
}

constexpr int TAIL_MAX_ROUNDS = 12;

template <int MODE, int CONV>
int launch(tbk_model* m, const HkArgs& a0, int grid) {
    hipStream_t s = m->stream;
    const size_t lds = 2 * STAGE_DOUBLES * sizeof(double);
    static std::atomic<bool> raised[TBK_MAX_DEVICES] = {};
    static std::atomic<bool> raised_split[TBK_MAX_DEVICES] = {};
    TBK_HIP(tbk_raise_lds_limit(reinterpret_cast<const void*>(&hk_dense_kernel<MODE, CONV, false>), 160 * 1024, raised));
    TBK_HIP(tbk_raise_lds_limit(reinterpret_cast<const void*>(&hk_dense_kernel<MODE, CONV, true>), 160 * 1024, raised_split));
    HkArgs a = a0;
    a.unit_grid = grid;
    const int slots = 2 * m->n_cu;
    const int n_stage = (int)(a.k2 / TBK_BK);
    const int units = grid * a.splits;
    const int full = units / slots * slots, tail = units - full;
    const int unit_stages = (n_stage + a.splits - 1) / a.splits;
    int sub = 1;
    if (full > 0 && tail > 0 && units < TAIL_MAX_ROUNDS * slots && unit_stages >= 8) {
        auto rounds = [&](int u) { return u <= slots / 2 ? 0.54 : (double)((u + slots - 1) / slots); };
        const double round_ms = 1.97 * unit_stages / 512.0;
        const double plain = rounds(tail) * round_ms;
        double best = std::min(0.9 * plain, plain - 0.03);
        for (int sp = 2; sp <= std::min(64, unit_stages / 4); ++sp) {
            const double cost = rounds(tail * sp) / sp * round_ms + sp * tail * 9e-5 + 0.01;
            if (cost < best) {
                best = cost;
                sub = sp;
            }
        }
    }
    const size_t base_bytes = a.splits > 1 ? (size_t)a.splits * a.p_rows * a.ncol_pad * 2 * sizeof(double) : 0;
    if (sub >= 2) {
        TBK_CHECK(m->ws_part.reserve(base_bytes + (size_t)sub * tail * TBK_BM * TBK_BNP * 2 * sizeof(double)));
        a.P = a.splits > 1 ? m->ws_part.as<double>() : nullptr;
        if (a.splits > 1)
            hipLaunchKernelGGL((hk_dense_kernel<MODE, CONV, true>), dim3(full), dim3(256), lds, s, a);
        else
            hipLaunchKernelGGL((hk_dense_kernel<MODE, CONV, false>), dim3(full), dim3(256), lds, s, a);
        TBK_HIP(hipGetLastError());
        HkArgs t = a;
        t.block_offset = full;
        t.p_tiles = tail;
        t.sub_splits = sub;
        t.P2 = reinterpret_cast<double*>(m->ws_part.as<char>() + base_bytes);
        hipLaunchKernelGGL((hk_dense_kernel<MODE, CONV, true>), dim3(tail, sub), dim3(256), lds, s, t);
        TBK_HIP(hipGetLastError());
        hipLaunchKernelGGL((hk_finish_tiles_kernel<MODE, CONV>), dim3(tail), dim3(256), 0, s, t);
        TBK_HIP(hipGetLastError());
    } else if (a.splits > 1) {
        hipLaunchKernelGGL((hk_dense_kernel<MODE, CONV, true>), dim3(units), dim3(256), lds, s, a);
        TBK_HIP(hipGetLastError());
    } else {
        hipLaunchKernelGGL((hk_dense_kernel<MODE, CONV, false>), dim3(grid), dim3(256), lds, s, a);
        TBK_HIP(hipGetLastError());
    }
    if (a.splits > 1) {
        const int64_t threads = a.nk * a.ncol_pad;
        hipLaunchKernelGGL((hk_finish_kernel<MODE, CONV>), dim3((unsigned)((threads + 255) / 256)), dim3(256), 0, s, a);
        TBK_HIP(hipGetLastError());
    }
    return TBK_OK;
}

HkArgs hk_args(const tbk_model* m, const tbk_operand_t& op, const double* d_A, int64_t nk, int64_t nk_pad, double* d_H) {
    HkArgs a;
    a.A = d_A;
    a.Bt = op.d_B;
    a.colmap = m->d_colmap;
    a.R = op.d_R;
    a.n_r = op.n_r;
    a.H = d_H;
    a.k2 = op.k2;
    a.nk = nk;
    a.nk_pad = nk_pad;
    a.ncol_pad = m->ncol_pad;
    a.n_orb = m->n_orb;
    a.dim = op.dim;
    a.nt_count = m->ncol_pad / TBK_BNP;
    return a;
}

int tile_grid(HkArgs& a, int mt_count) {
    a.mt_count = mt_count;
    a.xcd_rows = mt_count >= 32 ? 4 : 0;
    return mt_count >= 32 ? (mt_count + 7) / 8 * a.nt_count * 8 : mt_count * a.nt_count;
}

template <class F>
auto by_mode(int mode, int convention, F&& launch) {
    using std::integral_constant;
    if (mode == HK_TRI) return launch(integral_constant<int, HK_TRI>(), integral_constant<int, 2>());
    if (convention == 1) return launch(integral_constant<int, HK_FULL>(), integral_constant<int, 1>());
    return launch(integral_constant<int, HK_FULL>(), integral_constant<int, 2>());
}

template <int MODE, int CONV>
int launch_strassen(tbk_model* m, const tbk_operand_t& op, const HkArgs& a0) {
    hipStream_t s = m->stream;
    const size_t lds = 2 * STAGE_DOUBLES * sizeof(double);
    static std::atomic<bool> raised[TBK_MAX_DEVICES] = {};
    TBK_HIP(tbk_raise_lds_limit(reinterpret_cast<const void*>(&hk_dense_kernel<HK_TRI, 2, true>), 160 * 1024, raised));
    const int64_t mh = tbk_strassen_mh(a0.nk);
    const int half = a0.ncol_pad / 2;
    HkArgs a = hk_args(m, op, a0.A, mh, mh, a0.H);
    a.Bt = m->d_Bs;
    a.k2 = op.k2 / 2;
    a.ncol_pad = half;
    a.nt_count = half / TBK_BNP;
    const int grid = tile_grid(a, (int)(mh / TBK_BM));
    a.products = 1;
    a.splits = 7;
    a.unit_grid = grid;
    a.p_rows = mh;
    a.a_prod_stride = a.k2 * mh;
    a.b_prod_stride = a.k2 * half * 2;
    TBK_CHECK(m->ws_part.reserve((size_t)7 * mh * half * 2 * sizeof(double)));
    a.P = m->ws_part.as<double>();
    hipLaunchKernelGGL((hk_dense_kernel<HK_TRI, 2, true>), dim3(7 * grid), dim3(256), lds, s, a);
    TBK_HIP(hipGetLastError());
    HkArgs f = a0;
    f.P = a.P;
    const int64_t threads = mh * half;
    hipLaunchKernelGGL((hk_strassen_finish_kernel<MODE, CONV>), dim3((unsigned)((threads + 255) / 256)), dim3(256), 0, s, f, mh);
    TBK_HIP(hipGetLastError());
    m->counters[TBK_CNT_STRASSEN_LAUNCHES] += 1;
    return TBK_OK;
}

template <int MODE, int CONV>
int launch_strassen2(tbk_model* m, const tbk_operand_t& op, const HkArgs& a0) {
    hipStream_t s = m->stream;
    const size_t lds = 2 * STAGE_DOUBLES * sizeof(double);
    static std::atomic<bool> raised[TBK_MAX_DEVICES] = {};
    TBK_HIP(tbk_raise_lds_limit(reinterpret_cast<const void*>(&hk_dense_kernel<HK_TRI, 2, true>), 160 * 1024, raised));
    TBK_ARG(m->d_Bs2 != nullptr, "the operand blocks of the second Strassen level are missing");
    const int64_t mq = tbk_strassen_mq(a0.nk);
    const int quarter = a0.ncol_pad / 4;
    HkArgs a = hk_args(m, op, a0.A, mq, mq, a0.H);
    a.Bt = m->d_Bs2;
    a.k2 = op.k2 / 4;
    a.ncol_pad = quarter;
    a.nt_count = quarter / TBK_BNP;
    const int grid = tile_grid(a, (int)(mq / TBK_BM));
    a.products = 1;
    a.splits = 49;
    a.unit_grid = grid;
    a.p_rows = mq;
    a.a_prod_stride = a.k2 * mq;
    a.b_prod_stride = a.k2 * quarter * 2;
    TBK_CHECK(m->ws_part.reserve((size_t)49 * mq * quarter * 2 * sizeof(double)));
    a.P = m->ws_part.as<double>();
    hipLaunchKernelGGL((hk_dense_kernel<HK_TRI, 2, true>), dim3(49 * grid), dim3(256), lds, s, a);
    TBK_HIP(hipGetLastError());
    HkArgs f = a0;
    f.P = a.P;
    const int64_t threads = mq * quarter;
    hipLaunchKernelGGL((hk_strassen2_finish_kernel<MODE, CONV>), dim3((unsigned)((threads + 255) / 256)), dim3(256), 0, s, f, mq);
    TBK_HIP(hipGetLastError());
    m->counters[TBK_CNT_STRASSEN_LAUNCHES] += 1;
    m->counters[TBK_CNT_STRASSEN2_LAUNCHES] += 1;
    return TBK_OK;
}

int gemv_nkv(int64_t nk) {
    int nkv = 1;
    while (nkv < std::min<int64_t>(nk, 32)) nkv *= 2;
    return nkv;
}
int64_t gemv_strip_rows(int64_t k2, int64_t slices) {
    const int64_t n_pairs = k2 / 2;
    return (2 * ((n_pairs + slices - 1) / slices) + 15) / 16 * 16;
}

void gemv_plan(const tbk_model* m, int64_t k2, int64_t nk, int* slices_out, size_t* lds_out) {
    const int nblk = m->ncol_pad / 64;
    const int64_t n_pairs = k2 / 2;
    const size_t per_split = (size_t)nk * m->ncol_pad * 2 * sizeof(double);
    const int64_t cap = std::max<int64_t>(1, (int64_t)((size_t(256) << 20) / per_split));
    const int64_t wave_slots = (int64_t)m->n_cu * 8;
    int64_t slices = wave_slots / nblk;
    size_t lds = 80 * 1024;
    const int64_t rows_one_round = slices > 0 ? (k2 + slices - 1) / slices : k2 + 1;
    if (slices < 1 || nblk * slices * 10 < wave_slots * 9 || rows_one_round > 384 || slices > cap) {
        slices = std::max<int64_t>(k2 / 256, std::min<int64_t>(((int64_t)m->n_cu * 32 + nblk - 1) / nblk, n_pairs / 8));
        slices = std::max<int64_t>(1, std::min(cap, slices));
        lds = 16 * 1024;
    }
    slices = std::max<int64_t>(1, std::min(slices, n_pairs / 8));
    if (nblk * slices * 2 <= wave_slots) lds = 16 * 1024;
    if (lds < 64 * 1024) {
        const size_t need = (size_t)4 * gemv_strip_rows(k2, slices) * gemv_nkv(nk) * sizeof(double);
        if (need <= size_t(64) * 1024) lds = std::max(lds, need);
    }
    *slices_out = (int)slices;
    *lds_out = lds;
}

}

tbk_hk_plan_t tbk_hk_plan(const tbk_model* m, const tbk_operand_t& op, int64_t nk, bool caller_rows) {
    tbk_hk_plan_t p;
    p.op = op;
    p.nk = nk;
    p.nk_pad = (nk + TBK_BM - 1) / TBK_BM * TBK_BM;
    p.rows = m->kdotp ? HK_ROWS_MONOMIAL : HK_ROWS_PHASE;
    p.row_doubles = std::max<int64_t>(op.k2, 1) * p.nk_pad;
    if (m->sparse) {
        p.path = HK_PATH_CSR;
        return p;
    }
    if (nk >= 1 && op.k2 > 0 && (nk <= 32 || (nk <= 4096 && m->ncol_pad <= 256 && op.k2 < 16 * TBK_BK))) {
        gemv_plan(m, op.k2, nk, &p.splits, &p.lds);
        if (!caller_rows && !m->kdotp && op.d_R != nullptr && gemv_strip_rows(op.k2, p.splits) * gemv_nkv(nk) <= (int64_t)(p.lds / 32))
            p.rows = HK_ROWS_NONE;
        const bool tiny = p.rows == HK_ROWS_NONE && nk == 1 && m->ncol_pad <= 256 && op.k2 <= 4096;
        p.path = tiny ? HK_PATH_TINY : HK_PATH_GEMV;
        return p;
    }
    const int64_t tiles = (nk + TBK_BM - 1) / TBK_BM * (m->ncol_pad / TBK_BNP);
    if (m->strassen && m->d_Bs != nullptr && op.d_B == m->d_B && !m->kdotp && op.n_r_pad >= TBK_STRASSEN_MIN_NR &&
        nk >= TBK_STRASSEN_MIN_NK && tiles >= 2 * m->n_cu) {
        if (m->strassen_levels >= 2 && !m->bs2_skipped && nk >= TBK_STRASSEN2_MIN_NK && op.k2 % (4 * TBK_BK) == 0 &&
            m->ncol_pad % (4 * TBK_BNP) == 0) {
            p.path = HK_PATH_STRASSEN2;
            p.rows = HK_ROWS_STRASSEN2;
            p.row_doubles = 49 * (op.k2 / 4) * tbk_strassen_mq(nk);
            return p;
        }
        p.path = HK_PATH_STRASSEN;
        p.rows = HK_ROWS_STRASSEN;
        p.row_doubles = 7 * (op.k2 / 2) * tbk_strassen_mh(nk);
        return p;
    }
    p.path = HK_PATH_TILES;
    const int n_stage = (int)(op.k2 / TBK_BK);
    if (tiles < 2 * m->n_cu && n_stage >= 16) {
        int64_t splits = std::min<int64_t>((1280 + tiles / 2) / tiles, n_stage / 4);
        const size_t per_split = (size_t)p.nk_pad * m->ncol_pad * 2 * sizeof(double);
        splits = std::min<int64_t>(splits, (int64_t)((size_t(512) << 20) / per_split));
        if (splits > 1) p.splits = (int)splits;
    }
    return p;
}

int tbk_launch_hk_dense(tbk_model* m, const tbk_hk_plan_t& p, const double* d_A, int mode, int convention,
                        const double* d_k, const double* d_pos, double* d_H) {
    if (p.nk == 0) return TBK_OK;
    TBK_ARG(p.path != HK_PATH_CSR, "sparse models take tbk_launch_hk_csr");
    HkArgs a = hk_args(m, p.op, d_A, p.nk, p.nk_pad, d_H);
    a.kpts = d_k;
    a.pos = d_pos;
    const int grid = tile_grid(a, (int)((p.nk + TBK_BM - 1) / TBK_BM));
    if (m->h_k_inline != nullptr && p.nk == 1 && p.rows == HK_ROWS_NONE) {
        a.k_inline = 1;
        for (int d = 0; d < p.op.dim; ++d) a.k_val[d] = m->h_k_inline[d];
        a.pos_raw = m->d_pos_inline;
    }
    TBK_ARG(p.rows == HK_ROWS_NONE ? d_k != nullptr || a.k_inline : d_A != nullptr, "phase rows missing");
    TBK_ARG(convention != 1 || mode == HK_TRI || d_pos != nullptr || (a.k_inline && a.pos_raw != nullptr), "convention 1 needs the orbital phases");
    if (p.path == HK_PATH_TINY) {
        const int strip = (int)(((p.op.k2 / 2 + 3) / 4 * 2 + 15) / 16 * 16);
        const size_t lds = ((size_t)4 * strip + 4 * 64 * 2) * sizeof(double);
        StageTimer t(m, TBK_T_HK);
        return by_mode(mode, convention, [&](auto md, auto cv) {
            hipLaunchKernelGGL((hk_tiny_kernel<md, cv>), dim3((unsigned)(a.ncol_pad / 64)), dim3(256), lds, m->stream, a, strip);
            TBK_HIP(hipGetLastError());
            return TBK_OK;
        });
    }
    if (p.path == HK_PATH_GEMV) {
        TBK_CHECK(m->ws_part.reserve((size_t)p.nk * a.ncol_pad * 2 * sizeof(double) * p.splits));
        a.P = m->ws_part.as<double>();
        a.splits = p.splits;
        a.p_rows = p.nk;
        StageTimer t(m, TBK_T_HK);
        return by_mode(mode, convention, [&](auto md, auto cv) {
            TBK_HIP((launch_gemv<md, cv>(m, a, p.lds, m->stream)));
            return TBK_OK;
        });
    }
    if (p.path == HK_PATH_STRASSEN) {
        StageTimer t(m, TBK_T_HK);
        return by_mode(mode, convention, [&](auto md, auto cv) { return launch_strassen<md, cv>(m, p.op, a); });
    }
    if (p.path == HK_PATH_STRASSEN2) {
        StageTimer t(m, TBK_T_HK);
        return by_mode(mode, convention, [&](auto md, auto cv) { return launch_strassen2<md, cv>(m, p.op, a); });
    }
    if (p.splits > 1) {
        const size_t per_split = (size_t)p.nk_pad * a.ncol_pad * 2 * sizeof(double);
        TBK_CHECK(m->ws_part.reserve(per_split * p.splits));
        a.P = m->ws_part.as<double>();
        a.splits = p.splits;
        a.p_rows = p.nk_pad;
    }
    StageTimer t(m, TBK_T_HK);
    return by_mode(mode, convention, [&](auto md, auto cv) { return launch<md, cv>(m, a, grid); });
}

int tbk_launch_hk_dense_lines(tbk_model* m, const tbk_operand_t& op, const double* d_A, int64_t n_lines, int line_len,
                              int64_t b_stride, double* d_H) {
    if (n_lines == 0) return TBK_OK;
    TBK_ARG(line_len >= 1 && line_len <= TBK_BM, "a mesh line must fit one k tile");
    HkArgs a = hk_args(m, op, d_A, n_lines * line_len, TBK_BM, d_H);
    a.a_tile_stride = 0;
    a.b_tile_stride = b_stride;
    a.rows_per_tile = line_len;
    const int grid = tile_grid(a, (int)n_lines);
    StageTimer t(m, TBK_T_HK);
    return launch<HK_TRI, 2>(m, a, grid);
}
```

tbmodels_amd/csrc/tbk_internal.h:

```cpp
#pragma once

#include <hip/hip_runtime.h>
#include <rocblas/rocblas.h>

#include <atomic>
#include <cstdlib>
#include <cstdint>
#include <cstdio>
#include <functional>
#include <mutex>
#include <string>
#include <vector>

#include "tbk.h"

constexpr int TBK_BM = 128;
constexpr int TBK_BNP = 64;
constexpr int TBK_BK = 16;
constexpr int TBK_CT = 16;
constexpr int TBK_MAX_DIM = 8;

constexpr int32_t TBK_SLOT_PAIR = 0x8000;

void tbk_set_error(const char* fmt, ...);

#define TBK_HIP(expr)                                                                             \
    do {                                                                                          \
        hipError_t e_ = (expr);                                                                   \
        if (e_ != hipSuccess) {                                                                   \
            tbk_set_error("%s failed: %s (%s:%d)", #expr, hipGetErrorString(e_), __FILE__,        \
                          __LINE__);                                                              \
            return (e_ == hipErrorOutOfMemory) ? TBK_ERR_MEMORY : TBK_ERR_DEVICE;                 \
        }                                                                                         \
    } while (0)

#define TBK_ROCBLAS(expr)                                                                         \
    do {                                                                                          \
        rocblas_status s_ = (expr);                                                               \
        if (s_ != rocblas_status_success) {                                                       \
            tbk_set_error("%s failed: rocblas_status %d (%s:%d)", #expr, (int)s_, __FILE__,       \
                          __LINE__);                                                              \
            return (s_ == rocblas_status_memory_error) ? TBK_ERR_MEMORY : TBK_ERR_DEVICE;         \
        }                                                                                         \
    } while (0)

#define TBK_CHECK(expr)                                                                           \
    do {                                                                                          \
        int r_ = (expr);                                                                          \
        if (r_ != TBK_OK) return r_;                                                              \
    } while (0)

#define TBK_LOCK(m) std::lock_guard<std::recursive_mutex> tbk_lock_((m)->mu)

#define TBK_ARG(cond, msg)                                                                        \
    do {                                                                                          \
        if (!(cond)) {                                                                            \
            tbk_set_error("invalid argument: %s", msg);                                           \
            return TBK_ERR_ARGUMENT;                                                              \
        }                                                                                         \
    } while (0)

struct tbk_eig_env_t {
    bool band = true, band_split = true, band_xl = true, chase_window = true, reg128 = true, reg128_nw2 = true;
    int band_xl_from = 1024;
};
const tbk_eig_env_t& tbk_eig_env();

constexpr int TBK_MAX_DEVICES = 64;

using tbk_flag_row = std::atomic<bool>[TBK_MAX_DEVICES];
inline hipError_t tbk_raise_lds_limit(const void* kernel, int bytes, tbk_flag_row& done) {
    int dev = 0;
    hipError_t e = hipGetDevice(&dev);
    if (e != hipSuccess) return e;
    if (dev >= 0 && dev < TBK_MAX_DEVICES && done[dev].load(std::memory_order_acquire)) return hipSuccess;
    e = hipFuncSetAttribute(kernel, hipFuncAttributeMaxDynamicSharedMemorySize, bytes);
    if (e == hipSuccess && dev >= 0 && dev < TBK_MAX_DEVICES) done[dev].store(true, std::memory_order_release);
    return e;
}

struct DevBuf {
    void* ptr = nullptr;
    size_t bytes = 0;
    int reserve(size_t want);
    void release();
    template <class T>
    T* as() const {
        return static_cast<T*>(ptr);
    }
};

struct EventPair {
    hipEvent_t start, stop;
    int stage;
};

struct tbk_operand_t {
    int dim = 0;
    int64_t n_r = 0, n_r_pad = 0, k2 = 0;
    const int32_t* d_R = nullptr;
    const double* d_B = nullptr;
};

struct tbk_fold_plan_t {
    bool built = false;
    int dim = 0;
    int64_t n_r = 0;
    int64_t n_rho = 0, n_rho_pad = 0, k2 = 0;
    int64_t row_len = 0;
    int capacity = 0;
    std::vector<int32_t> h_R2;
    int32_t* d_R2 = nullptr;
    int64_t* d_lptr = nullptr;
    int32_t* d_lrec = nullptr;
    int32_t* d_rcomp = nullptr;
    double* d_B2 = nullptr;
    double* d_table = nullptr;
    int64_t table_entries = 0;
    tbk_fold_plan_t* sub = nullptr;
    double* slot(int s) const { return d_B2 + (size_t)s * k2 * row_len; }
    tbk_operand_t operand(int s) const { return {dim - 1, n_rho, n_rho_pad, k2, d_R2, slot(s)}; }
};

struct tbk_model {
    std::recursive_mutex mu;
    int device = 0;
    int n_cu = 256;
    int dim = 0;
    int n_orb = 0;
    int64_t n_r = 0;
    bool sparse = false;
    bool kdotp = false;

    int64_t n_r_pad = 0;
    int64_t k2 = 0;
    int ncol = 0;
    int ncol_pad = 0;
    int32_t* d_R = nullptr;
    int32_t* d_colmap = nullptr;
    int32_t* d_powers = nullptr;

    double* d_B = nullptr;
    double* d_Bs = nullptr;
    double* d_Bs2 = nullptr;
    bool bs2_skipped = false;

    int64_t nnz_rec = 0;
    int64_t* d_cptr = nullptr;
    int32_t* d_rec_r = nullptr;
    double* d_rec_v = nullptr;
    int sched_kt = 0;
    int64_t sched_steps = 0;
    int64_t* d_sptr = nullptr;
    int32_t* d_srec_r = nullptr;
    double* d_srec_v = nullptr;

    int64_t staged_bytes = 0;

    std::vector<int32_t> h_R;
    tbk_fold_plan_t fold[TBK_MAX_DIM];
    bool fold_enabled = true;
    bool strassen = true;
    int strassen_levels = 2;
    int64_t counters[TBK_CNT_COUNT] = {0, 0, 0, 0, 0, 0};

    int eigensolver = TBK_EIG_AUTO;
    int64_t k_chunk = 0;
    bool timing = false;

    hipStream_t stream = nullptr;
    hipStream_t stream_eig = nullptr;
    hipStream_t stream_ql = nullptr;
    hipStream_t stream_xl[3] = {nullptr, nullptr, nullptr};
    hipEvent_t ev_xl[4] = {nullptr, nullptr, nullptr, nullptr};
    hipEvent_t ev_hk[2] = {nullptr, nullptr};
    hipEvent_t ev_tri[2] = {nullptr, nullptr};
    hipEvent_t ev_out[2] = {nullptr, nullptr};
    hipEvent_t ev_ql[2] = {nullptr, nullptr};
    hipEvent_t ev_sync = nullptr;
    rocblas_handle blas = nullptr;
    DevBuf ws_phase;
    DevBuf ws_H;
    DevBuf ws_H2;
    DevBuf ws_E;
    DevBuf ws_E2;
    DevBuf ws_info;
    DevBuf ws_k;
    DevBuf ws_pos;
    DevBuf ws_orb;
    DevBuf ws_out;
    DevBuf ws_out2;
    DevBuf ws_flag;
    void* h_stage = nullptr;
    size_t h_stage_bytes = 0;
    DevBuf ws_part;
    DevBuf ws_kfold;
    DevBuf ws_kline;
    DevBuf ws_band;
    DevBuf ws_bandmat[2];
    const double* h_k_inline = nullptr;
    const double* d_pos_inline = nullptr;
    std::vector<double> pos_cache;
    DevBuf ws_posraw;
    DevBuf ws_xl;
    std::function<int(int64_t c0, int64_t nkc, hipEvent_t done)> chunk_done;
    std::vector<EventPair> events;
    double t_ms[TBK_T_COUNT] = {0, 0, 0, 0};
    int64_t t_n[TBK_T_COUNT] = {0, 0, 0, 0};
};

inline tbk_operand_t tbk_staged_operand(const tbk_model* m) { return {m->dim, m->n_r, m->n_r_pad, m->k2, m->d_R, m->d_B}; }

struct tbk_kdotp {
    tbk_model* core = nullptr;
};

void tbk_range_push(const char* name);
void tbk_range_pop();

struct StageTimer {
    tbk_model* m;
    EventPair ev;
    bool on;
    hipStream_t stream;
    StageTimer(tbk_model* m_, int stage, hipStream_t s = nullptr);
    ~StageTimer();
};

enum HkMode { HK_TRI = 0, HK_FULL = 1 };

constexpr int64_t TBK_STRASSEN_MIN_NR = 1024;
constexpr int64_t TBK_STRASSEN_MIN_NK = 4096;
inline bool tbk_strassen_model(bool sparse, bool kdotp, int64_t n_r) { return !sparse && !kdotp && n_r >= TBK_STRASSEN_MIN_NR; }
inline int64_t tbk_strassen_mh(int64_t nk) { return (((nk + 1) / 2) + TBK_BM - 1) / TBK_BM * TBK_BM; }
constexpr int64_t TBK_STRASSEN2_MIN_NK = 8192;
inline int64_t tbk_strassen_mq(int64_t nk) { return (((nk + 3) / 4) + TBK_BM - 1) / TBK_BM * TBK_BM; }

enum HkPath {
    HK_PATH_CSR,
    HK_PATH_TINY,
    HK_PATH_GEMV,
    HK_PATH_STRASSEN,
    HK_PATH_STRASSEN2,
    HK_PATH_TILES,
};
enum HkRows {
    HK_ROWS_NONE,
    HK_ROWS_PHASE,
    HK_ROWS_MONOMIAL,
    HK_ROWS_STRASSEN,
    HK_ROWS_STRASSEN2,
};
struct tbk_hk_plan_t {
    tbk_operand_t op;
    HkPath path = HK_PATH_TILES;
    HkRows rows = HK_ROWS_PHASE;
    int64_t nk = 0;
    int64_t nk_pad = 0;
    int64_t row_doubles = 0;
    int splits = 1;
    size_t lds = 0;
};
tbk_hk_plan_t tbk_hk_plan(const tbk_model* m, const tbk_operand_t& op, int64_t nk, bool caller_rows);

int64_t choose_chunk(tbk_model* m, int64_t nk, bool with_eig);
int fill_rows(tbk_model* m, const tbk_hk_plan_t& plan, const double* d_k);
int build_h(tbk_model* m, const tbk_hk_plan_t& plan, int mode, int convention, const double* d_k, const double* d_pos, double* d_H);

int tbk_launch_phase_strassen(tbk_model* m, const tbk_operand_t& op, const double* d_k, int64_t nk, double* d_As);
int tbk_launch_phase_strassen2(tbk_model* m, const tbk_operand_t& op, const double* d_k, int64_t nk, double* d_As2);
int tbk_launch_phase(tbk_model* m, const tbk_operand_t& op, const double* d_k, int64_t nk, int64_t nk_pad, double* d_A);
int tbk_launch_orbital_phases(tbk_model* m, const double* d_k, const double* d_pos, int64_t nk, double* d_orb);
int tbk_launch_monomials(hipStream_t s, const int32_t* d_powers, int dim, int64_t n_p,
                         int64_t n_p_pad, const double* d_k, int64_t nk, int64_t nk_pad,
                         double* d_A);

int tbk_stage_dense(tbk_model* m, const double* d_hop_raw);
int tbk_stage_kdotp(tbk_model* m, const double* d_coeff_raw);
int tbk_stage_strassen(tbk_model* m);
size_t tbk_strassen2_bytes(const tbk_model* m);
int tbk_stage_strassen2(tbk_model* m);

int tbk_launch_hk_dense(tbk_model* m, const tbk_hk_plan_t& plan, const double* d_A, int mode, int convention,
                        const double* d_k, const double* d_pos, double* d_H);

int tbk_launch_hk_dense_lines(tbk_model* m, const tbk_operand_t& op, const double* d_A, int64_t n_lines, int line_len, int64_t b_stride,
                              double* d_H);

int tbk_launch_hk_csr(tbk_model* m, const double* d_A, int64_t nk, int64_t nk_pad, int mode,
                      int convention, const double* d_k, const double* d_pos, double* d_H);

int tbk_csr_tile_kpoints(int64_t n_r);
void tbk_csr_schedule(int ncol, int kt, const std::vector<int64_t>& cptr, const std::vector<int32_t>& rec_r, const std::vector<double>& rec_v,
                      std::vector<int64_t>& sptr, std::vector<int32_t>& srec_r, std::vector<double>& srec_v);

int tbk_eig_batched(tbk_model* m, double* d_H, int64_t nk, double* d_E);

int tbk_eigh_check_arguments(int64_t nk, int convention, const double* pos);

constexpr int ST_MAXN = 512;
constexpr int BAND_ONE_WG_MAXN = 1024;
constexpr int BAND_LDS_CHASE_MAXN = 512;
enum EigFamily { EIG_ROCSOLVER, EIG_REGISTER, EIG_ONE_STAGE, EIG_TWO_STAGE };
enum EigChase { EIG_CHASE_LDS, EIG_CHASE_WINDOW16, EIG_CHASE_WINDOW32, EIG_CHASE_GLOBAL };
struct tbk_eig_plan_t {
    int n = 0;
    int64_t call_nk = 0;
    EigFamily family = EIG_ROCSOLVER;
    bool split_on = false;
    bool reg128 = false;
    bool via128 = false;
    bool reg128_nw2 = false;
    bool chain = false;
    bool chain_by_size = false;
    bool wide = false;
    bool fused = false;
    EigChase chase = EIG_CHASE_LDS;
    bool chase_buffer = false;
    bool bisect = false;
    int bisect_lanes = 1;
    size_t band_stride = 0, ws_band = 0, ws_bandmat = 0, ws_xl = 0;
    bool own() const { return family != EIG_ROCSOLVER; }
};
tbk_eig_plan_t tbk_eig_plan(int n_orb, int eigensolver, int64_t call_nk, int method = TBK_REDUCE_AUTO);
int tbk_eig_check_option(const tbk_model* m);
bool tbk_eig_small_supported(int n);
bool tbk_eig_band_supported(int n);
int tbk_eig_xl_groups(const tbk_eig_plan_t& plan, int64_t nk);
size_t tbk_eig_scratch_per_k(const tbk_model* m);
int tbk_eig_reserve(tbk_model* m, const tbk_eig_plan_t& plan, int64_t max_nk, int bandmats);
int tbk_eig_reduce(tbk_model* m, const tbk_eig_plan_t& plan, hipStream_t s, double* d_H, int64_t nk, double* d_de, void* d_band = nullptr);

int tbk_launch_tridiag_stream(tbk_model* m, const tbk_eig_plan_t& plan, hipStream_t s, double* d_H, int64_t nk, double* d_de);
int tbk_launch_bisect(tbk_model* m, const tbk_eig_plan_t& plan, hipStream_t s, const double* d_de, int64_t nk, double* d_E);

size_t tbk_band_scratch_per_matrix(int n);
size_t tbk_band_bytes_per_matrix(int n, bool chase_buffer);
int tbk_launch_band_reduce(tbk_model* m, const tbk_eig_plan_t& plan, hipStream_t s, double* d_H, int64_t nk, void* d_vw, void* d_band,
                           double* d_de_fused = nullptr);
int tbk_launch_band_chase(tbk_model* m, const tbk_eig_plan_t& plan, hipStream_t s, const void* d_band, int64_t nk, double* d_de);

int tbk_launch_tridiag(tbk_model* m, const tbk_eig_plan_t& plan, hipStream_t s, double* d_H, int64_t nk, double* d_de);
int tbk_launch_tridiag_reg128(const tbk_eig_plan_t& plan, hipStream_t s, double* d_H, int n, int64_t nk, double* d_D, double* d_E, int64_t h_stride, int ldd, int off);
int tbk_launch_tridiag_tail64(const tbk_eig_plan_t& plan, hipStream_t s, double* d_H, int64_t nk, double* d_D, double* d_E, int n_full);
int tbk_launch_ql(tbk_model* m, hipStream_t s, const double* d_de, int64_t nk, double* d_E, bool beside_ql = false);

std::vector<int64_t> run_schedule(const std::vector<int64_t>& runs, int64_t chunk);

struct LineInfo {
    bool ok = false;
    int e2 = -1;
    int64_t L = 0;
    int64_t body = 0;
    int64_t n_lines = 0;
};

struct tbk_folded_call {
    tbk_folded_call(tbk_model* m, const double* d_k, const double* h_k, int64_t nk);
    bool folds() const { return f >= 0; }
    std::vector<int64_t> runs;
    int begin();
    int build(int64_t c0, int64_t nkc, double* d_H);

private:
    int run_operand(size_t r, tbk_operand_t* op);
    int piece_plane(const tbk_operand_t& op, int64_t lo, int64_t hi, double* d_Hp);
    int fold_body(const tbk_operand_t& from, tbk_fold_plan_t& plan2, const LineInfo& li, int64_t a0, int64_t n, int slot0);
    int contract_lines(tbk_fold_plan_t& plan2, const LineInfo& li, int64_t a0, int64_t n, double* d_Hp);
    int piece(const tbk_operand_t& op, int64_t lo, int64_t hi, double* d_Hp);
    int batched(int64_t c0, int64_t nkc, double* d_H, bool* done);

    tbk_model* m;
    const double* d_k;
    const double* h_k;
    int64_t nk;
    int f = -1;
    int dim = 0, dim1 = 0;
    size_t nn2 = 0;
    tbk_fold_plan_t* plan1 = nullptr;
    std::vector<int> reduced;
    int64_t group_lo = -1;
    double* d_k2 = nullptr;
};
void tbk_fold_release(tbk_model* m);

int tbk_run_mfma_f64_peak(double* tflops);
```

Measured before the change: 1.156 million k-points/s.

## Fold previous chunk's Strassen combine into next chunk's GEMM as side units

For consecutive Strassen-path chunks in the eigenvalue pipeline, the product buffers of one chunk are parked in a second workspace. Their combine step then runs as extra 'side' thread blocks inside the next chunk's Hk GEMM launch, with nontemporal stores to H. This removes a separate finish-kernel launch per chunk and lets the memory-bound combine overlap with compute-bound GEMM blocks. In exchange it doubles the product workspace, which shrinks the chunk size, and makes the cross-stream event scheduling more complex.

After: 1.162 million k-points/s (median of 6 runs). No clear change (+0.5%).

```diff
diff --git a/include/tbk.h b/include/tbk.h
--- a/include/tbk.h
+++ b/include/tbk.h
@@ -27,7 +27,8 @@
     TBK_OPT_TIMING = 3,
     TBK_OPT_FOLD = 4,
     TBK_OPT_STRASSEN = 5,
-    TBK_OPT_STRASSEN_LEVELS = 6
+    TBK_OPT_STRASSEN_LEVELS = 6,
+    TBK_OPT_HK_SIDE_UNITS = 7
 };
 
 const char* tbk_version(void);
@@ -50,7 +51,8 @@
        TBK_CNT_LIBRARY_CALLS = 3,
        TBK_CNT_STRASSEN_LAUNCHES = 4,
        TBK_CNT_STRASSEN2_LAUNCHES = 5,
-       TBK_CNT_COUNT = 6 };
+       TBK_CNT_HK_SIDE_LAUNCHES = 6,
+       TBK_CNT_COUNT = 7 };
 int tbk_model_counter(tbk_model* m, int counter, int64_t* value);
 
 
diff --git a/tbmodels_amd/_lib.py b/tbmodels_amd/_lib.py
--- a/tbmodels_amd/_lib.py
+++ b/tbmodels_amd/_lib.py
@@ -19,6 +19,8 @@
 TBK_REDUCE_AUTO, TBK_REDUCE_ONE_STAGE, TBK_REDUCE_TWO_STAGE = 0, 1, 2
 TBK_CNT_EIGENVAL_CALLS, TBK_CNT_FOLDED_CALLS, TBK_CNT_FOLDED_KPOINTS, TBK_CNT_LIBRARY_CALLS, TBK_CNT_STRASSEN_LAUNCHES = 0, 1, 2, 3, 4
 TBK_CNT_STRASSEN2_LAUNCHES = 5
+TBK_OPT_HK_SIDE_UNITS = 7
+TBK_CNT_HK_SIDE_LAUNCHES = 6
 TBK_T_PHASE, TBK_T_HK, TBK_T_EIG, TBK_T_QL, TBK_T_COUNT = 0, 1, 2, 3, 4
 STAGE_NAMES = ("phase", "hk", "eig", "ql")
 
diff --git a/tbmodels_amd/csrc/tbk_api.hip b/tbmodels_amd/csrc/tbk_api.hip
--- a/tbmodels_amd/csrc/tbk_api.hip
+++ b/tbmodels_amd/csrc/tbk_api.hip
@@ -358,7 +358,7 @@
     for (void* p : ptrs)
         if (p) (void)hipFree(p);
     DevBuf* bufs[] = {&m->ws_phase, &m->ws_H, &m->ws_E,   &m->ws_E2,
-                      &m->ws_info,  &m->ws_k, &m->ws_pos, &m->ws_out, &m->ws_out2, &m->ws_flag, &m->ws_orb, &m->ws_part, &m->ws_kfold, &m->ws_kline, &m->ws_band, &m->ws_bandmat[0], &m->ws_bandmat[1], &m->ws_H2, &m->ws_xl, &m->ws_posraw};
+                      &m->ws_info,  &m->ws_k, &m->ws_pos, &m->ws_out, &m->ws_out2, &m->ws_flag, &m->ws_orb, &m->ws_part, &m->ws_part2, &m->ws_kfold, &m->ws_kline, &m->ws_band, &m->ws_bandmat[0], &m->ws_bandmat[1], &m->ws_H2, &m->ws_xl, &m->ws_posraw};
     for (DevBuf* b : bufs) b->release();
     tbk_fold_release(m);
     delete m;
@@ -389,6 +389,10 @@
             TBK_ARG(value == 1 || value == 2, "Strassen levels must be 1 or 2");
             m->strassen_levels = (int)value;
             return TBK_OK;
+        case TBK_OPT_HK_SIDE_UNITS:
+            TBK_ARG(value == 0 || value == 1, "side units are 0 or 1");
+            m->hk_side_units = value != 0;
+            return TBK_OK;
         default:
             tbk_set_error("unknown option %d", option);
             return TBK_ERR_ARGUMENT;
@@ -415,7 +419,7 @@
     size_t free_b = 0, total_b = 0;
     if (hipMemGetInfo(&free_b, &total_b) != hipSuccess) free_b = size_t(8) << 30;
     free_b += m->ws_H.bytes + m->ws_H2.bytes + m->ws_phase.bytes + m->ws_band.bytes + m->ws_bandmat[0].bytes + m->ws_bandmat[1].bytes +
-              m->ws_E.bytes + m->ws_xl.bytes + m->ws_part.bytes;
+              m->ws_E.bytes + m->ws_xl.bytes + m->ws_part.bytes + m->ws_part2.bytes;
     const bool mid = n > 64 && n <= 256;
     int64_t budget = std::min<int64_t>((int64_t)(free_b / 4), int64_t(mid ? 64 : n > 64 ? 24 : 6) << 30);
     int64_t chunk = budget / per_k / TBK_BM * TBK_BM;
@@ -423,6 +427,7 @@
     if (n < 64) cap *= std::min<int64_t>(32, (64 / n) * (64 / n));
     chunk = std::max<int64_t>(TBK_BM, std::min<int64_t>(chunk, cap));
     tbk_hk_plan_t plan = tbk_hk_plan(m, tbk_staged_operand(m), std::min(chunk, nk), false);
+    const int n_part = with_eig && tbk_hk_side_units(m) && nk >= 2 * TBK_STRASSEN_MIN_NK ? 2 : 1;
     if (plan.path == HK_PATH_STRASSEN2) {
         size_t free2 = free_b;
         if (m->d_Bs2 == nullptr) {
@@ -431,14 +436,14 @@
             else free2 -= blocks;
         }
         if (!m->bs2_skipped) {
-            const int64_t per_k_s = per_k + m->k2 * 8 * 33 / 16 + (int64_t)m->ncol_pad * 16 * 49 / 16;
+            const int64_t per_k_s = per_k + m->k2 * 8 * 33 / 16 + (int64_t)m->ncol_pad * 16 * 49 / 16 * n_part;
             const int64_t fit = (int64_t)(free2 / 4) / per_k_s / TBK_BM * TBK_BM;
             chunk = std::max<int64_t>(TBK_BM, std::min(chunk, fit));
         }
         plan = tbk_hk_plan(m, tbk_staged_operand(m), std::min(chunk, nk), false);
     }
     if (plan.path == HK_PATH_STRASSEN) {
-        const int64_t per_k_s = per_k + m->k2 * 8 * 3 / 4 + (int64_t)m->ncol_pad * 16 * 7 / 4;
+        const int64_t per_k_s = per_k + m->k2 * 8 * 3 / 4 + (int64_t)m->ncol_pad * 16 * 7 / 4 * n_part;
         const int64_t fit = (int64_t)(free_b / 4) / per_k_s / TBK_BM * TBK_BM;
         chunk = std::max<int64_t>(TBK_BM, std::min(chunk, fit));
     }
@@ -531,8 +536,10 @@
                                   const HBuilder* builder = nullptr, const std::vector<int64_t>* runs = nullptr) {
     int64_t rows_ready_for = -1;
     tbk_hk_plan_t rows_plan;
+    std::vector<tbk_hk_plan_t> chain;
+    int64_t chain_at = 0;
     const auto prepare_rows = [&](int64_t c0, int64_t nkc) -> int {
-        rows_plan = tbk_hk_plan(m, tbk_staged_operand(m), nkc, false);
+        rows_plan = chain.empty() ? tbk_hk_plan(m, tbk_staged_operand(m), nkc, false) : chain[chain_at];
         if (rows_plan.rows != HK_ROWS_NONE) TBK_CHECK(fill_rows(m, rows_plan, d_k + c0 * m->dim));
         rows_ready_for = c0;
         return TBK_OK;
@@ -573,41 +580,70 @@
         }
         return TBK_OK;
     }
-    int64_t prev_c0 = 0, prev_nkc = 0, c0 = 0;
+    std::vector<int64_t> start(n_chunks, 0);
+    for (int64_t c = 1; c < n_chunks; ++c) start[c] = start[c - 1] + sched[c - 1];
+    if (!builder) {
+        for (int64_t c = 0; c < n_chunks; ++c) chain.push_back(tbk_hk_plan(m, tbk_staged_operand(m), sched[c], false));
+        const size_t part_bytes = tbk_hk_plan_chain(m, chain);
+        if (part_bytes > 0) {
+            for (const tbk_hk_plan_t& p : chain)
+                if (p.rows == HK_ROWS_STRASSEN2) TBK_CHECK(tbk_stage_strassen2(m));
+            TBK_CHECK(m->ws_part.reserve(part_bytes));
+            TBK_CHECK(m->ws_part2.reserve(part_bytes));
+        }
+    }
+    const auto reduce_and_ql = [&](int64_t j) -> int {
+        const int b = (int)(j & 1);
+        TBK_HIP(hipStreamWaitEvent(m->stream_eig, m->ev_hk[b], 0));
+        if (j >= 2 && h_overlap) TBK_HIP(hipStreamWaitEvent(m->stream_eig, m->ev_ql[b], 0));
+        TBK_CHECK(tbk_eig_reduce(m, plan, m->stream_eig, d_Hbuf[b], sched[j], debuf[b]->as<double>(), two_stage ? m->ws_bandmat[b].ptr : nullptr));
+        TBK_HIP(hipEventRecord(m->ev_tri[b], m->stream_eig));
+        if (j >= 1) {
+            TBK_HIP(hipStreamWaitEvent(m->stream_ql, m->ev_hk[b], 0));
+            if (h_overlap) TBK_HIP(hipStreamWaitEvent(m->stream_ql, m->ev_tri[b ^ 1], 0));
+            TBK_CHECK(launch_tridiag_eigenvalues(m, plan, m->stream_ql, debuf[b ^ 1]->as<double>(), sched[j - 1],
+                                                 d_E + (size_t)start[j - 1] * n, false, false,
+                                                 two_stage ? m->ws_bandmat[b ^ 1].ptr : nullptr));
+            TBK_HIP(hipEventRecord(m->ev_ql[b ^ 1], m->stream_ql));
+            if (m->chunk_done) TBK_CHECK(m->chunk_done(start[j - 1], sched[j - 1], m->ev_ql[b ^ 1]));
+        }
+        return TBK_OK;
+    };
+    int64_t reduced = -1;
     for (int64_t c = 0; c < n_chunks; ++c) {
         const int b = (int)(c & 1);
-        const int64_t nkc = sched[c];
-        double* d_de = debuf[b]->as<double>();
-        d_H = d_Hbuf[b];
+        const int64_t nkc = sched[c], c0 = start[c];
+        const tbk_hk_plan_t* hp = builder ? nullptr : &chain[c];
+        chain_at = c;
+        const bool carries = hp && hp->carry_nk > 0, parks = hp && hp->park;
+        const int64_t j = carries ? c - 1 : c;
         if (c >= 1) {
             if (!builder) TBK_CHECK(prepare_rows(c0, nkc));
-            if (!h_overlap)
-                TBK_HIP(hipStreamWaitEvent(m->stream, m->ev_tri[b ^ 1], 0));
-            else if (c >= 2)
+            if (!h_overlap) {
+                if (reduced >= 0) TBK_HIP(hipStreamWaitEvent(m->stream, m->ev_tri[reduced & 1], 0));
+            } else if (c >= 2) {
                 TBK_HIP(hipStreamWaitEvent(m->stream, m->ev_tri[b], 0));
-            if (c >= 2 && !h_overlap) TBK_HIP(hipStreamWaitEvent(m->stream, m->ev_ql[b], 0));
-        }
-        TBK_CHECK(build(c0, nkc, d_H));
-        TBK_HIP(hipEventRecord(m->ev_hk[b], m->stream));
-
-        TBK_HIP(hipStreamWaitEvent(m->stream_eig, m->ev_hk[b], 0));
-        if (c >= 2 && h_overlap) TBK_HIP(hipStreamWaitEvent(m->stream_eig, m->ev_ql[b], 0));
-        TBK_CHECK(tbk_eig_reduce(m, plan, m->stream_eig, d_H, nkc, d_de, two_stage ? m->ws_bandmat[b].ptr : nullptr));
-        TBK_HIP(hipEventRecord(m->ev_tri[b], m->stream_eig));
-
-        if (c >= 1) {
-            TBK_HIP(hipStreamWaitEvent(m->stream_ql, m->ev_hk[b], 0));
-            if (h_overlap) TBK_HIP(hipStreamWaitEvent(m->stream_ql, m->ev_tri[b ^ 1], 0));
-            TBK_CHECK(launch_tridiag_eigenvalues(m, plan, m->stream_ql, debuf[b ^ 1]->as<double>(), prev_nkc,
-                                                 d_E + (size_t)prev_c0 * n, false, false,
-                                                 two_stage ? m->ws_bandmat[b ^ 1].ptr : nullptr));
-            TBK_HIP(hipEventRecord(m->ev_ql[b ^ 1], m->stream_ql));
-            if (m->chunk_done) TBK_CHECK(m->chunk_done(prev_c0, prev_nkc, m->ev_ql[b ^ 1]));
-        }
-        prev_c0 = c0;
-        prev_nkc = nkc;
-        c0 += nkc;
-    }
+            }
+            if (j >= 2 && !h_overlap) TBK_HIP(hipStreamWaitEvent(m->stream, m->ev_ql[j & 1], 0));
+        }
+        TBK_CHECK(build(c0, nkc, d_Hbuf[b]));
+        if (carries) {
+            TBK_HIP(hipEventRecord(m->ev_hk[b ^ 1], m->stream));
+            TBK_CHECK(reduce_and_ql(c - 1));
+            reduced = c - 1;
+        }
+        if (parks && !hp->carried) {
+            if (reduced >= 0) TBK_HIP(hipStreamWaitEvent(m->stream, m->ev_tri[reduced & 1], 0));
+            if (c >= 2) TBK_HIP(hipStreamWaitEvent(m->stream, m->ev_ql[b], 0));
+            TBK_CHECK(tbk_launch_hk_combine(m, *hp, HK_TRI, 2, d_Hbuf[b]));
+        }
+        if (!parks || !hp->carried) {
+            TBK_HIP(hipEventRecord(m->ev_hk[b], m->stream));
+            TBK_CHECK(reduce_and_ql(c));
+            reduced = c;
+        }
+    }
+    const int64_t prev_c0 = start[n_chunks - 1], prev_nkc = sched[n_chunks - 1];
     {
         const int b = (int)((n_chunks - 1) & 1);
         TBK_CHECK(launch_tridiag_eigenvalues(m, plan, m->stream_eig, debuf[b]->as<double>(), prev_nkc,
diff --git a/tbmodels_amd/csrc/tbk_hk_dense.hip b/tbmodels_amd/csrc/tbk_hk_dense.hip
--- a/tbmodels_amd/csrc/tbk_hk_dense.hip
+++ b/tbmodels_amd/csrc/tbk_hk_dense.hip
@@ -52,11 +52,24 @@
     double k_val[TBK_MAX_DIM] = {};
     int k_inline = 0;
     const double* pos_raw = nullptr;
+    int side_groups = 0;
+    int side_period = 0;
+    int side_levels = 0;
+    int side_cols = 0;
+    int side_per = 0;
+    int64_t side_m = 0, side_nk = 0;
+    const double* side_P = nullptr;
 };
 
 __device__ __forceinline__ double hk_kcomp(const HkArgs& a, int64_t kq, int d) { return a.k_inline ? a.k_val[d] : a.kpts[kq * a.dim + d]; }
 
-template <int MODE, int CONV>
+template <bool NT>
+__device__ __forceinline__ void store_d2(double* at, d2 v) {
+    if (NT) __builtin_nontemporal_store(v, reinterpret_cast<d2*>(at));
+    else *reinterpret_cast<d2*>(at) = v;
+}
+
+template <int MODE, int CONV, bool NT = false>
 __device__ __forceinline__ void store_element(const HkArgs& a, int64_t kq, int oi, int oj, double re, double im) {
     if (CONV == 1 && oi != oj) {
         d2 ei, ej;
@@ -81,20 +94,20 @@
         re = t;
     }
     double* hk = a.H + (size_t)kq * a.n_orb * a.n_orb * 2;
-    *reinterpret_cast<d2*>(hk + ((size_t)oi * a.n_orb + oj) * 2) = (d2){re, im};
-    if (MODE == HK_FULL && oi != oj) *reinterpret_cast<d2*>(hk + ((size_t)oj * a.n_orb + oi) * 2) = (d2){re, -im};
-}
-
-template <int MODE, int CONV>
+    store_d2<NT>(hk + ((size_t)oi * a.n_orb + oj) * 2, (d2){re, im});
+    if (MODE == HK_FULL && oi != oj) store_d2<NT>(hk + ((size_t)oj * a.n_orb + oi) * 2, (d2){re, -im});
+}
+
+template <int MODE, int CONV, bool NT = false>
 __device__ __forceinline__ void store_slot(const HkArgs& a, int64_t kq, int32_t slot, double v0, double v1) {
     const int oi = slot >> 16, oj = slot & 0x7fff;
     if (slot & TBK_SLOT_PAIR) {
         double* hk = a.H + (size_t)kq * a.n_orb * a.n_orb * 2;
-        *reinterpret_cast<d2*>(hk + ((size_t)oi * a.n_orb + oi) * 2) = (d2){v0, 0.0};
-        *reinterpret_cast<d2*>(hk + ((size_t)oj * a.n_orb + oj) * 2) = (d2){v1, 0.0};
+        store_d2<NT>(hk + ((size_t)oi * a.n_orb + oi) * 2, (d2){v0, 0.0});
+        store_d2<NT>(hk + ((size_t)oj * a.n_orb + oj) * 2, (d2){v1, 0.0});
         return;
     }
-    store_element<MODE, CONV>(a, kq, oi, oj, v0, v1);
+    store_element<MODE, CONV, NT>(a, kq, oi, oj, v0, v1);
 }
 
 __device__ __forceinline__ bool tile_of_block(const HkArgs& a, int b, int& mt, int& nt) {
@@ -125,11 +138,105 @@
     return true;
 }
 
+template <bool NT>
+__device__ __forceinline__ d2 load_d2(const d2* at) {
+    return NT ? __builtin_nontemporal_load(at) : *at;
+}
+
+template <int MODE, int CONV, bool NT>
+__device__ __forceinline__ void strassen_combine_at(const HkArgs& a, const double* P, int ncol_pad, int64_t nk, int64_t mh, int64_t idx) {
+    const int half = ncol_pad / 2;
+    const int e = (int)(idx % half);
+    const int64_t kq = idx / half;
+    if (kq >= mh) return;
+    const size_t blk = (size_t)mh * half;
+    const d2* mp = reinterpret_cast<const d2*>(P) + (size_t)kq * half + e;
+    const d2 m1 = load_d2<NT>(mp), m2 = load_d2<NT>(mp + blk), m3 = load_d2<NT>(mp + 2 * blk), m4 = load_d2<NT>(mp + 3 * blk),
+             m5 = load_d2<NT>(mp + 4 * blk), m6 = load_d2<NT>(mp + 5 * blk), m7 = load_d2<NT>(mp + 6 * blk);
+    const d2 c11 = ((m1 + m4) - m5) + m7;
+    const d2 c12 = m3 + m5;
+    const d2 c21 = m2 + m4;
+    const d2 c22 = ((m1 - m2) + m3) + m6;
+    const int32_t ij0 = a.colmap[e], ij1 = a.colmap[e + half];
+    if (kq < nk) {
+        if (ij0 >= 0) store_slot<MODE, CONV, NT>(a, kq, ij0, c11[0], c11[1]);
+        if (ij1 >= 0) store_slot<MODE, CONV, NT>(a, kq, ij1, c12[0], c12[1]);
+    }
+    if (kq + mh < nk) {
+        if (ij0 >= 0) store_slot<MODE, CONV, NT>(a, kq + mh, ij0, c21[0], c21[1]);
+        if (ij1 >= 0) store_slot<MODE, CONV, NT>(a, kq + mh, ij1, c22[0], c22[1]);
+    }
+}
+
+template <int MODE, int CONV, bool NT>
+__device__ __forceinline__ void strassen2_combine_at(const HkArgs& a, const double* P, int ncol_pad, int64_t nk, int64_t mq, int64_t idx) {
+    const int quarter = ncol_pad / 4;
+    const int e = (int)(idx % quarter);
+    const int64_t kq = idx / quarter;
+    if (kq >= mq) return;
+    const size_t blk = (size_t)mq * quarter;
+    const d2* mp = reinterpret_cast<const d2*>(P) + (size_t)kq * quarter + e;
+    d2 c[2][2][2][2];
+#pragma unroll
+    for (int p1 = 0; p1 < 7; ++p1) {
+        const d2* q = mp + (size_t)(7 * p1) * blk;
+        const d2 m1 = load_d2<NT>(q), m2 = load_d2<NT>(q + blk), m3 = load_d2<NT>(q + 2 * blk), m4 = load_d2<NT>(q + 3 * blk),
+                 m5 = load_d2<NT>(q + 4 * blk), m6 = load_d2<NT>(q + 5 * blk), m7 = load_d2<NT>(q + 6 * blk);
+        const d2 in[2][2] = {{((m1 + m4) - m5) + m7, m3 + m5}, {m2 + m4, ((m1 - m2) + m3) + m6}};
+#pragma unroll
+        for (int a2 = 0; a2 < 2; ++a2)
+#pragma unroll
+            for (int c2 = 0; c2 < 2; ++c2) {
+                const d2 v = in[a2][c2];
+                if (p1 == 0) c[0][0][a2][c2] = v, c[1][1][a2][c2] = v;
+                if (p1 == 1) c[1][0][a2][c2] = v, c[1][1][a2][c2] -= v;
+                if (p1 == 2) c[0][1][a2][c2] = v, c[1][1][a2][c2] += v;
+                if (p1 == 3) c[0][0][a2][c2] += v, c[1][0][a2][c2] += v;
+                if (p1 == 4) c[0][0][a2][c2] -= v, c[0][1][a2][c2] += v;
+                if (p1 == 5) c[1][1][a2][c2] += v;
+                if (p1 == 6) c[0][0][a2][c2] += v;
+            }
+    }
+#pragma unroll
+    for (int cq = 0; cq < 4; ++cq) {
+        const int32_t ij = a.colmap[e + cq * quarter];
+        if (ij < 0) continue;
+#pragma unroll
+        for (int aq = 0; aq < 4; ++aq) {
+            const int64_t kout = kq + aq * mq;
+            if (kout >= nk) continue;
+            const d2 v = c[aq >> 1][cq >> 1][aq & 1][cq & 1];
+            store_slot<MODE, CONV, NT>(a, kout, ij, v[0], v[1]);
+        }
+    }
+}
+
+template <int MODE, int CONV>
+__device__ __forceinline__ void side_unit(const HkArgs& a, int su) {
+    const int64_t total = a.side_m * a.side_cols;
+    int64_t idx = (int64_t)su * a.side_per * 256 + threadIdx.x;
+    if (a.side_levels == 2) {
+        for (int it = 0; it < a.side_per && idx < total; ++it, idx += 256)
+            strassen2_combine_at<MODE, CONV, true>(a, a.side_P, a.side_cols * 4, a.side_nk, a.side_m, idx);
+    } else {
+        for (int it = 0; it < a.side_per && idx < total; ++it, idx += 256)
+            strassen_combine_at<MODE, CONV, true>(a, a.side_P, a.side_cols * 2, a.side_nk, a.side_m, idx);
+    }
+}
+
 template <int MODE, int CONV, bool SPLIT>
 __global__ void __launch_bounds__(256, 2) hk_dense_kernel(const HkArgs a) {
     extern __shared__ __attribute__((aligned(16))) double smem[];
 
-    const int unit = (int)blockIdx.x + a.block_offset;
+    int unit = (int)blockIdx.x + a.block_offset;
+    if (SPLIT && a.side_groups > 0) {
+        const int g = (int)blockIdx.x >> 3, t = g / a.side_period;
+        if (t < a.side_groups && g - t * a.side_period == a.side_period - 1) {
+            side_unit<MODE, CONV>(a, t * 8 + ((int)blockIdx.x & 7));
+            return;
+        }
+        unit -= 8 * min(t, a.side_groups);
+    }
     const int split_y = SPLIT ? unit / a.unit_grid : 0;
     int mt_idx, nt_idx;
     if (!tile_of_block(a, SPLIT ? unit - split_y * a.unit_grid : unit, mt_idx, nt_idx)) return;
@@ -464,70 +571,12 @@
 
 template <int MODE, int CONV>
 __global__ void __launch_bounds__(256) hk_strassen_finish_kernel(const HkArgs a, int64_t mh) {
-    const int half = a.ncol_pad / 2;
-    const int64_t idx = (int64_t)blockIdx.x * 256 + threadIdx.x;
-    const int e = (int)(idx % half);
-    const int64_t kq = idx / half;
-    if (kq >= mh) return;
-    const size_t blk = (size_t)mh * half;
-    const d2* mp = reinterpret_cast<const d2*>(a.P) + (size_t)kq * half + e;
-    const d2 m1 = mp[0], m2 = mp[blk], m3 = mp[2 * blk], m4 = mp[3 * blk], m5 = mp[4 * blk], m6 = mp[5 * blk], m7 = mp[6 * blk];
-    const d2 c11 = ((m1 + m4) - m5) + m7;
-    const d2 c12 = m3 + m5;
-    const d2 c21 = m2 + m4;
-    const d2 c22 = ((m1 - m2) + m3) + m6;
-    const int32_t ij0 = a.colmap[e], ij1 = a.colmap[e + half];
-    if (kq < a.nk) {
-        if (ij0 >= 0) store_slot<MODE, CONV>(a, kq, ij0, c11[0], c11[1]);
-        if (ij1 >= 0) store_slot<MODE, CONV>(a, kq, ij1, c12[0], c12[1]);
-    }
-    if (kq + mh < a.nk) {
-        if (ij0 >= 0) store_slot<MODE, CONV>(a, kq + mh, ij0, c21[0], c21[1]);
-        if (ij1 >= 0) store_slot<MODE, CONV>(a, kq + mh, ij1, c22[0], c22[1]);
-    }
+    strassen_combine_at<MODE, CONV, false>(a, a.P, a.ncol_pad, a.nk, mh, (int64_t)blockIdx.x * 256 + threadIdx.x);
 }
 
 template <int MODE, int CONV>
 __global__ void __launch_bounds__(256) hk_strassen2_finish_kernel(const HkArgs a, int64_t mq) {
-    const int quarter = a.ncol_pad / 4;
-    const int64_t idx = (int64_t)blockIdx.x * 256 + threadIdx.x;
-    const int e = (int)(idx % quarter);
-    const int64_t kq = idx / quarter;
-    if (kq >= mq) return;
-    const size_t blk = (size_t)mq * quarter;
-    const d2* mp = reinterpret_cast<const d2*>(a.P) + (size_t)kq * quarter + e;
-    d2 c[2][2][2][2];
-#pragma unroll
-    for (int p1 = 0; p1 < 7; ++p1) {
-        const d2* q = mp + (size_t)(7 * p1) * blk;
-        const d2 m1 = q[0], m2 = q[blk], m3 = q[2 * blk], m4 = q[3 * blk], m5 = q[4 * blk], m6 = q[5 * blk], m7 = q[6 * blk];
-        const d2 in[2][2] = {{((m1 + m4) - m5) + m7, m3 + m5}, {m2 + m4, ((m1 - m2) + m3) + m6}};
-#pragma unroll
-        for (int a2 = 0; a2 < 2; ++a2)
-#pragma unroll
-            for (int c2 = 0; c2 < 2; ++c2) {
-                const d2 v = in[a2][c2];
-                if (p1 == 0) c[0][0][a2][c2] = v, c[1][1][a2][c2] = v;
-                if (p1 == 1) c[1][0][a2][c2] = v, c[1][1][a2][c2] -= v;
-                if (p1 == 2) c[0][1][a2][c2] = v, c[1][1][a2][c2] += v;
-                if (p1 == 3) c[0][0][a2][c2] += v, c[1][0][a2][c2] += v;
-                if (p1 == 4) c[0][0][a2][c2] -= v, c[0][1][a2][c2] += v;
-                if (p1 == 5) c[1][1][a2][c2] += v;
-                if (p1 == 6) c[0][0][a2][c2] += v;
-            }
-    }
-#pragma unroll
-    for (int cq = 0; cq < 4; ++cq) {
-        const int32_t ij = a.colmap[e + cq * quarter];
-        if (ij < 0) continue;
-#pragma unroll
-        for (int aq = 0; aq < 4; ++aq) {
-            const int64_t kout = kq + aq * mq;
-            if (kout >= a.nk) continue;
-            const d2 v = c[aq >> 1][cq >> 1][aq & 1][cq & 1];
-            store_slot<MODE, CONV>(a, kout, ij, v[0], v[1]);
-        }
-    }
+    strassen2_combine_at<MODE, CONV, false>(a, a.P, a.ncol_pad, a.nk, mq, (int64_t)blockIdx.x * 256 + threadIdx.x);
 }
 
 template <int MODE, int CONV>
@@ -728,8 +777,48 @@
     return launch(integral_constant<int, HK_FULL>(), integral_constant<int, 2>());
 }
 
-template <int MODE, int CONV>
-int launch_strassen(tbk_model* m, const tbk_operand_t& op, const HkArgs& a0) {
+DevBuf& product_buffer(tbk_model* m, const tbk_hk_plan_t& p) { return p.pbuf ? m->ws_part2 : m->ws_part; }
+
+constexpr int SIDE_PER = 64;
+int carry_combine(tbk_model* m, const tbk_hk_plan_t& p, HkArgs& a, int blocks) {
+    if (p.carry_nk <= 0) return blocks;
+    const int levels = p.carry_path == HK_PATH_STRASSEN2 ? 2 : 1;
+    a.side_levels = levels;
+    a.side_nk = p.carry_nk;
+    a.side_m = levels == 2 ? tbk_strassen_mq(p.carry_nk) : tbk_strassen_mh(p.carry_nk);
+    a.side_cols = m->ncol_pad / (levels == 2 ? 4 : 2);
+    a.side_P = (p.pbuf ? m->ws_part : m->ws_part2).as<double>();
+    const int64_t total = a.side_m * a.side_cols;
+    const int64_t groups_p = blocks / 8;
+    int64_t groups_s = (total + (int64_t)256 * SIDE_PER * 8 - 1) / ((int64_t)256 * SIDE_PER * 8);
+    groups_s = std::max<int64_t>(1, std::min(groups_s, groups_p / 2));
+    a.side_groups = (int)groups_s;
+    a.side_per = (int)((total + 256 * 8 * groups_s - 1) / (256 * 8 * groups_s));
+    a.side_period = (int)std::max<int64_t>(2, (groups_p - groups_p / 8) / groups_s);
+    m->counters[TBK_CNT_HK_SIDE_LAUNCHES] += 1;
+    return blocks + 8 * a.side_groups;
+}
+
+template <int MODE, int CONV>
+int strassen_combine(tbk_model* m, const tbk_hk_plan_t& p, const HkArgs& a0) {
+    HkArgs f = a0;
+    f.P = product_buffer(m, p).as<double>();
+    if (p.path == HK_PATH_STRASSEN2) {
+        const int64_t mq = tbk_strassen_mq(a0.nk);
+        const int64_t threads = mq * (a0.ncol_pad / 4);
+        hipLaunchKernelGGL((hk_strassen2_finish_kernel<MODE, CONV>), dim3((unsigned)((threads + 255) / 256)), dim3(256), 0, m->stream, f, mq);
+    } else {
+        const int64_t mh = tbk_strassen_mh(a0.nk);
+        const int64_t threads = mh * (a0.ncol_pad / 2);
+        hipLaunchKernelGGL((hk_strassen_finish_kernel<MODE, CONV>), dim3((unsigned)((threads + 255) / 256)), dim3(256), 0, m->stream, f, mh);
+    }
+    TBK_HIP(hipGetLastError());
+    return TBK_OK;
+}
+
+template <int MODE, int CONV>
+int launch_strassen(tbk_model* m, const tbk_hk_plan_t& p, const HkArgs& a0) {
+    const tbk_operand_t& op = p.op;
     hipStream_t s = m->stream;
     const size_t lds = 2 * STAGE_DOUBLES * sizeof(double);
     static std::atomic<bool> raised[TBK_MAX_DEVICES] = {};
@@ -748,21 +837,19 @@
     a.p_rows = mh;
     a.a_prod_stride = a.k2 * mh;
     a.b_prod_stride = a.k2 * half * 2;
-    TBK_CHECK(m->ws_part.reserve((size_t)7 * mh * half * 2 * sizeof(double)));
-    a.P = m->ws_part.as<double>();
-    hipLaunchKernelGGL((hk_dense_kernel<HK_TRI, 2, true>), dim3(7 * grid), dim3(256), lds, s, a);
-    TBK_HIP(hipGetLastError());
-    HkArgs f = a0;
-    f.P = a.P;
-    const int64_t threads = mh * half;
-    hipLaunchKernelGGL((hk_strassen_finish_kernel<MODE, CONV>), dim3((unsigned)((threads + 255) / 256)), dim3(256), 0, s, f, mh);
+    TBK_CHECK(product_buffer(m, p).reserve((size_t)7 * mh * half * 2 * sizeof(double)));
+    a.P = product_buffer(m, p).as<double>();
+    const int blocks = carry_combine(m, p, a, 7 * grid);
+    hipLaunchKernelGGL((hk_dense_kernel<HK_TRI, 2, true>), dim3(blocks), dim3(256), lds, s, a);
     TBK_HIP(hipGetLastError());
     m->counters[TBK_CNT_STRASSEN_LAUNCHES] += 1;
-    return TBK_OK;
-}
-
-template <int MODE, int CONV>
-int launch_strassen2(tbk_model* m, const tbk_operand_t& op, const HkArgs& a0) {
+    if (p.park) return TBK_OK;
+    return strassen_combine<MODE, CONV>(m, p, a0);
+}
+
+template <int MODE, int CONV>
+int launch_strassen2(tbk_model* m, const tbk_hk_plan_t& p, const HkArgs& a0) {
+    const tbk_operand_t& op = p.op;
     hipStream_t s = m->stream;
     const size_t lds = 2 * STAGE_DOUBLES * sizeof(double);
     static std::atomic<bool> raised[TBK_MAX_DEVICES] = {};
@@ -782,18 +869,15 @@
     a.p_rows = mq;
     a.a_prod_stride = a.k2 * mq;
     a.b_prod_stride = a.k2 * quarter * 2;
-    TBK_CHECK(m->ws_part.reserve((size_t)49 * mq * quarter * 2 * sizeof(double)));
-    a.P = m->ws_part.as<double>();
-    hipLaunchKernelGGL((hk_dense_kernel<HK_TRI, 2, true>), dim3(49 * grid), dim3(256), lds, s, a);
-    TBK_HIP(hipGetLastError());
-    HkArgs f = a0;
-    f.P = a.P;
-    const int64_t threads = mq * quarter;
-    hipLaunchKernelGGL((hk_strassen2_finish_kernel<MODE, CONV>), dim3((unsigned)((threads + 255) / 256)), dim3(256), 0, s, f, mq);
+    TBK_CHECK(product_buffer(m, p).reserve((size_t)49 * mq * quarter * 2 * sizeof(double)));
+    a.P = product_buffer(m, p).as<double>();
+    const int blocks = carry_combine(m, p, a, 49 * grid);
+    hipLaunchKernelGGL((hk_dense_kernel<HK_TRI, 2, true>), dim3(blocks), dim3(256), lds, s, a);
     TBK_HIP(hipGetLastError());
     m->counters[TBK_CNT_STRASSEN_LAUNCHES] += 1;
     m->counters[TBK_CNT_STRASSEN2_LAUNCHES] += 1;
-    return TBK_OK;
+    if (p.park) return TBK_OK;
+    return strassen_combine<MODE, CONV>(m, p, a0);
 }
 
 int gemv_nkv(int64_t nk) {
@@ -877,6 +961,34 @@
     return p;
 }
 
+size_t tbk_hk_plan_chain(const tbk_model* m, std::vector<tbk_hk_plan_t>& plans) {
+    size_t bytes = 0;
+    if (!tbk_hk_side_units(m)) return bytes;
+    const auto strassen = [](const tbk_hk_plan_t& p) { return p.path == HK_PATH_STRASSEN || p.path == HK_PATH_STRASSEN2; };
+    for (size_t c = 0; c + 1 < plans.size(); ++c) {
+        if (!strassen(plans[c]) || !strassen(plans[c + 1])) continue;
+        plans[c].park = plans[c].carried = true;
+        plans[c + 1].park = true;
+        plans[c + 1].carry_path = plans[c].path;
+        plans[c + 1].carry_nk = plans[c].nk;
+    }
+    for (size_t c = 0; c < plans.size(); ++c) {
+        if (!plans[c].park) continue;
+        plans[c].pbuf = (int)(c & 1);
+        const tbk_hk_plan_t& p = plans[c];
+        const size_t elems = p.path == HK_PATH_STRASSEN2 ? (size_t)49 * tbk_strassen_mq(p.nk) * (m->ncol_pad / 4)
+                                                         : (size_t)7 * tbk_strassen_mh(p.nk) * (m->ncol_pad / 2);
+        bytes = std::max(bytes, elems * 2 * sizeof(double));
+    }
+    return bytes;
+}
+
+int tbk_launch_hk_combine(tbk_model* m, const tbk_hk_plan_t& p, int mode, int convention, double* d_H) {
+    TBK_ARG(p.park && (p.path == HK_PATH_STRASSEN || p.path == HK_PATH_STRASSEN2) && mode == HK_TRI && convention == 2, "no parked products to combine");
+    const HkArgs a = hk_args(m, p.op, nullptr, p.nk, p.nk_pad, d_H);
+    return by_mode(mode, convention, [&](auto md, auto cv) { return strassen_combine<md, cv>(m, p, a); });
+}
+
 int tbk_launch_hk_dense(tbk_model* m, const tbk_hk_plan_t& p, const double* d_A, int mode, int convention,
                         const double* d_k, const double* d_pos, double* d_H) {
     if (p.nk == 0) return TBK_OK;
@@ -892,6 +1004,8 @@
     }
     TBK_ARG(p.rows == HK_ROWS_NONE ? d_k != nullptr || a.k_inline : d_A != nullptr, "phase rows missing");
     TBK_ARG(convention != 1 || mode == HK_TRI || d_pos != nullptr || (a.k_inline && a.pos_raw != nullptr), "convention 1 needs the orbital phases");
+    TBK_ARG(!(p.park || p.carry_nk > 0) || ((p.path == HK_PATH_STRASSEN || p.path == HK_PATH_STRASSEN2) && mode == HK_TRI && convention == 2),
+            "parked products and side units belong to the Strassen chunks of an eigenvalue pipeline");
     if (p.path == HK_PATH_TINY) {
         const int strip = (int)(((p.op.k2 / 2 + 3) / 4 * 2 + 15) / 16 * 16);
         const size_t lds = ((size_t)4 * strip + 4 * 64 * 2) * sizeof(double);
@@ -915,11 +1029,11 @@
     }
     if (p.path == HK_PATH_STRASSEN) {
         StageTimer t(m, TBK_T_HK);
-        return by_mode(mode, convention, [&](auto md, auto cv) { return launch_strassen<md, cv>(m, p.op, a); });
+        return by_mode(mode, convention, [&](auto md, auto cv) { return launch_strassen<md, cv>(m, p, a); });
     }
     if (p.path == HK_PATH_STRASSEN2) {
         StageTimer t(m, TBK_T_HK);
-        return by_mode(mode, convention, [&](auto md, auto cv) { return launch_strassen2<md, cv>(m, p.op, a); });
+        return by_mode(mode, convention, [&](auto md, auto cv) { return launch_strassen2<md, cv>(m, p, a); });
     }
     if (p.splits > 1) {
         const size_t per_split = (size_t)p.nk_pad * a.ncol_pad * 2 * sizeof(double);
diff --git a/tbmodels_amd/csrc/tbk_internal.h b/tbmodels_amd/csrc/tbk_internal.h
--- a/tbmodels_amd/csrc/tbk_internal.h
+++ b/tbmodels_amd/csrc/tbk_internal.h
@@ -162,7 +162,8 @@
     bool fold_enabled = true;
     bool strassen = true;
     int strassen_levels = 2;
-    int64_t counters[TBK_CNT_COUNT] = {0, 0, 0, 0, 0, 0};
+    bool hk_side_units = true;
+    int64_t counters[TBK_CNT_COUNT] = {0, 0, 0, 0, 0, 0, 0};
 
     int eigensolver = TBK_EIG_AUTO;
     int64_t k_chunk = 0;
@@ -194,6 +195,7 @@
     void* h_stage = nullptr;
     size_t h_stage_bytes = 0;
     DevBuf ws_part;
+    DevBuf ws_part2;
     DevBuf ws_kfold;
     DevBuf ws_kline;
     DevBuf ws_band;
@@ -260,8 +262,14 @@
     int64_t row_doubles = 0;
     int splits = 1;
     size_t lds = 0;
+    bool park = false, carried = false;
+    int pbuf = 0;
+    HkPath carry_path = HK_PATH_TILES;
+    int64_t carry_nk = 0;
 };
 tbk_hk_plan_t tbk_hk_plan(const tbk_model* m, const tbk_operand_t& op, int64_t nk, bool caller_rows);
+size_t tbk_hk_plan_chain(const tbk_model* m, std::vector<tbk_hk_plan_t>& plans);
+inline bool tbk_hk_side_units(const tbk_model* m) { return m->hk_side_units && m->n_orb <= 64; }
 
 int64_t choose_chunk(tbk_model* m, int64_t nk, bool with_eig);
 int fill_rows(tbk_model* m, const tbk_hk_plan_t& plan, const double* d_k);
@@ -283,6 +291,8 @@
 
 int tbk_launch_hk_dense(tbk_model* m, const tbk_hk_plan_t& plan, const double* d_A, int mode, int convention,
                         const double* d_k, const double* d_pos, double* d_H);
+
+int tbk_launch_hk_combine(tbk_model* m, const tbk_hk_plan_t& plan, int mode, int convention, double* d_H);
 
 int tbk_launch_hk_dense_lines(tbk_model* m, const tbk_operand_t& op, const double* d_A, int64_t n_lines, int line_len, int64_t b_stride,
                               double* d_H);
```
